# brunohs1993/Nanokappa

Measured on AMD Instinct MI355X. Metric: phonon-steps/sec (whole node), higher is better.
Workload: dtype f64

## Files before the change

include/nanokappa_hip.h:

```cpp
#ifndef NANOKAPPA_HIP_H
#define NANOKAPPA_HIP_H
#include <stdint.h>

#ifdef __cplusplus
extern "C" {
#endif

typedef struct nk_ctx nk_ctx;

enum nk_status {
    NK_OK = 0,
    NK_ERR_HIP = -1,
    NK_ERR_ARG = -2,
    NK_ERR_CAPACITY = -3,
    NK_ERR_COMM = -4,
    NK_ERR_NODEVICE = -5
};

typedef struct {
    int32_t Q, J, NT;
    const double *omega;
    const double *group_vel;
    const double *T_grid;
    const double *lifetime;
// ... 54 lines not shown
    const int64_t *n_leaving;
} nk_reservoirs;

typedef struct {
    int32_t Fr;
    const int32_t *facet;
    const double *specularity;
    const uint8_t *true_spec;
    const int32_t *spec_map;
    const double *roulette;
    const int32_t *degen_j2;
} nk_rough;

typedef struct {
    double dt;
    int32_t norm_fixed;
    double particle_density;
    int32_t T_ref_local;
    double T_ref;
    int32_t flux_every;
    int32_t contains_every;
    int32_t track_ids;
} nk_params;

typedef struct {
    double *T_sv;
    double *E_sv;
    double *E_raw;
    double *N_sv;
    double *flux_raw;
    double *N_leaving;
    double *res_energy;
    double *res_flux;
    double *N_emitted;
} nk_tally;

typedef struct {
    double step_kernel_ms;
    double emit_kernel_ms;
    double events_kernel_ms;
    double total_ms;
    int64_t slots;
    int64_t live;
    int64_t regrows;
    int64_t halts;
    int64_t tau_rebuilds;
    int64_t batches;
    int64_t emit_fused;
    int64_t place_tries;
    double place_gbps;
    double place_worst_gbps;
    int64_t box_store;
} nk_timing;

int nk_device_count(void);
int nk_mesh_crossings(int device, int64_t n_rays, const double *origins, const double *dirs, int64_t n_faces, const double *v0,
                      const double *e1, const double *e2, int skip_self, int32_t *counts);
int nk_create(nk_ctx **out, int device_id, uint64_t seed);
void nk_destroy(nk_ctx *ctx);
const char *nk_last_error(const nk_ctx *ctx);

int nk_set_material(nk_ctx *ctx, const nk_material *m);
int nk_set_mesh(nk_ctx *ctx, const nk_mesh *m);
int nk_set_subvolumes(nk_ctx *ctx, const nk_subvols *s, const double *T_sv_init );
int nk_set_reservoirs(nk_ctx *ctx, const nk_reservoirs *r);
int nk_set_rough(nk_ctx *ctx, const nk_rough *r);
int nk_set_params(nk_ctx *ctx, const nk_params *p);

int nk_reserve(nk_ctx *ctx, int64_t capacity);
int nk_upload_particles(nk_ctx *ctx, int64_t N, const double *x, const double *y, const double *z,
                        const int32_t *mode, const double *occ, const double *n_ts, const int32_t *facet,
                        const uint64_t *pid, uint64_t pid_offset);
int nk_init_boundaries(nk_ctx *ctx);
int nk_init_particles(nk_ctx *ctx, int64_t N, int64_t capacity, uint64_t pid_lo, const int32_t *unique_modes, int64_t n_unique,
                      const int64_t *sv_first);
int nk_tally_state(nk_ctx *ctx, double *E_raw, double *N_sv, double *flux_raw);
int nk_step(nk_ctx *ctx, int32_t nsteps, nk_tally *out);
int nk_download_particles(nk_ctx *ctx, int64_t capacity, double *x, double *y, double *z, int32_t *mode,
                          double *occ, double *n_ts, int32_t *facet, uint64_t *pid, int64_t *N_out);
int nk_get_subvol_temperature(nk_ctx *ctx, double *T_sv );
int nk_set_subvol_temperature(nk_ctx *ctx, const double *T_sv );
int nk_get_step(nk_ctx *ctx, int64_t *step);
int nk_get_timing(nk_ctx *ctx, nk_timing *t);

int nk_comm_unique_id(void *id128 );
int nk_comm_init(nk_ctx *ctx, const void *id128, int rank, int nranks);
typedef struct {
    int32_t rank, nranks;
    int32_t comm_rank, comm_nranks;
    int32_t device;
    int32_t selftest_ok;
    double selftest_sum;
    char pci_bus_id[32];
} nk_comm_report;
int nk_comm_info(nk_ctx *ctx, nk_comm_report *out);
int nk_comm_allreduce(nk_ctx *ctx, double *inout, int64_t n);

int nk_set_bands(nk_ctx *ctx, int32_t nbands, const int32_t *band_of_mode);
int nk_get_band_rows(nk_ctx *ctx, double *F, double *N, int64_t *steps, int32_t cap, int32_t *nrows);
int nk_tally_bands_state(nk_ctx *ctx, double *F, double *N);

typedef struct {
    double lo[3], h[3];
    int32_t n[3];
    int32_t every;
    int32_t flags;
    int64_t capacity;
} nk_field;
#define NK_FIELD_GLOBAL 1
#define NK_FIELD_TEST_SMALL_BOUND 2
int nk_set_field(nk_ctx *ctx, const nk_field *f);
int nk_get_field(nk_ctx *ctx, double *N, double *E, double *F, int64_t *samples, int64_t *clamped, int32_t reset);
int nk_tally_field_state(nk_ctx *ctx, int64_t *raw, int64_t *clamped);
typedef struct {
    int32_t n[3], every;
    int64_t ncells;
    int32_t k_E, k_F;
    double B_E, B_F;
    int64_t capacity;
    int64_t bytes;
    int32_t lds_path;
    int32_t on;
} nk_field_report;
int nk_field_info(nk_ctx *ctx, nk_field_report *out);

int nk_set_field_groups(nk_ctx *ctx, int32_t ngroups, const int32_t *group_of_mode);
int nk_get_field_groups(nk_ctx *ctx, double *N, double *E, double *F, int64_t *samples, int64_t *ungrouped, int32_t reset);
int nk_tally_field_groups_state(nk_ctx *ctx, int64_t *raw, int64_t *clamped, int64_t *ungrouped);
typedef struct {
    int32_t G;
    int32_t lds_path;
    int64_t lines;
    int64_t bytes;
    int32_t k_E, k_F;
    int64_t permutes;
    int32_t on, pad_;
} nk_field_groups_report;
int nk_field_groups_info(nk_ctx *ctx, nk_field_groups_report *out);

typedef struct {
    int64_t ncells, pairs;
    int32_t k_A, k_P;
    double seconds;
} nk_solid_report;
int nk_cell_solid_volume(int device, int64_t n_faces, const double *tri , const double lo[3],
                         const double h[3], const int32_t n[3], double *V , nk_solid_report *rep );
const char *nk_solid_last_error(void);

typedef struct {
    int32_t every;
    int32_t flags;
    int64_t capacity;
} nk_modes;
#define NK_MODES_GLOBAL 1
#define NK_MODES_TEST_SMALL_BOUND 2
int nk_set_modes(nk_ctx *ctx, const nk_modes *m);
int nk_get_modes(nk_ctx *ctx, double *N, double *E, int64_t *samples, int64_t *skipped, int32_t reset);
int nk_tally_modes_state(nk_ctx *ctx, int64_t *N, int64_t *E);
typedef struct {
    int32_t every, k_E;
    double B_E;
    int64_t capacity;
    int64_t bytes;
    int32_t owner_path;
    int32_t on;
} nk_modes_report;
// ... 192 lines not shown
```

nanokappa_amd/csrc/nk_engine.hip:

```cpp
#include <hip/hip_runtime.h>
#include <dlfcn.h>
#include <math.h>
#include <stdio.h>
#include <stdlib.h>
#include <string.h>
#include <algorithm>
#include <functional>
#include <map>
#include <mutex>
#include <queue>
#include <string>
#include <type_traits>
#include <chrono>
#include <time.h>
#include <vector>

#include <rccl/rccl.h>

#include "../../include/nanokappa_hip.h"
#include "nk_kernels.h"
#include "nk_field.h"
#include "nk_modes.h"
#include "nk_group.h"
#include "nk_freepath.h"
#include "nk_freecols.h"
#include "nk_kinetic.h"
#ifndef NK_PLAIN_IN_ENGINE
extern template __global__ void k_sweep<1, false, false, false, false, true, 1>(NkDev, uint32_t, int, int);
extern template __global__ void k_sweep<1, false, false, false, false, true, 2>(NkDev, uint32_t, int, int);
extern template __global__ void k_sweep<1, false, false, false, false, false, 1>(NkDev, uint32_t, int, int);
extern template __global__ void k_sweep<1, false, false, false, false, false, 2>(NkDev, uint32_t, int, int);
extern template __global__ void k_sweep<1, false, false, false, false, true, 1, true>(NkDev, uint32_t, int, int);
extern template __global__ void k_sweep<1, false, false, false, false, true, 2, true>(NkDev, uint32_t, int, int);
extern template __global__ void k_sweep<1, false, false, false, false, false, 1, true>(NkDev, uint32_t, int, int);
extern template __global__ void k_sweep<1, false, false, false, false, false, 2, true>(NkDev, uint32_t, int, int);
#endif

struct NkRccl {
    void *lib = nullptr;
    ncclResult_t (*GetUniqueId)(ncclUniqueId *) = nullptr;
    ncclResult_t (*CommInitRank)(ncclComm_t *, int, ncclUniqueId, int) = nullptr;
    ncclResult_t (*AllReduce)(const void *, void *, size_t, ncclDataType_t, ncclRedOp_t, ncclComm_t, hipStream_t) = nullptr;
    ncclResult_t (*CommDestroy)(ncclComm_t) = nullptr;
    ncclResult_t (*CommCount)(const ncclComm_t, int *) = nullptr;
    ncclResult_t (*CommUserRank)(const ncclComm_t, int *) = nullptr;
    ncclResult_t (*CommAbort)(ncclComm_t) = nullptr;
};

static thread_local std::string g_create_error;

struct nk_ctx {
    int device = 0;
    hipStream_t stream = nullptr;
    std::string err;
    NkDev d;
    std::vector<void *> allocs;
    std::vector<void *> pallocs;
    void *store_buf = nullptr;
    size_t store_pad = 0;
    bool store_pid = false;
    bool store_nts = true;
    bool mesh_box = false;
    bool box_forbidden = false;
    int32_t *anomalies = nullptr;
    bool have_material = false, have_mesh = false, have_sv = false, have_params = false;
    int64_t step = 0;
    bool pending_relax = false;
    int g_sweep = 0;
    std::vector<hipEvent_t> evpool;
    NkSweepKind g_sweep_kind = {};
    size_t g_sweep_lds = 0;
    int layout_key = -1;
    std::vector<double> h_enter_prob;
    int64_t spec_M = 0;
    double *spec_v = nullptr, *spec_om = nullptr, *spec_dl = nullptr, *spec_svx = nullptr;
    int32_t *spec_rank = nullptr;
    double spec_vmax = 0.0;
    NkSpecMode *spec_modes = nullptr;
    int32_t *spec_in = nullptr, *spec_out = nullptr;
    unsigned long long *spec_count = nullptr;
    double *ks_kv = nullptr, *ks_mat = nullptr;
    double ks_tol[3] = {0, 0, 0};
    int64_t ks_Q = 0;
    int64_t spec_cap = 0;
    int64_t spec_last = 0;
    int rb_Fr = 0;
    double *rb_k2 = nullptr, *rb_nin = nullptr, *rb_eta = nullptr, *rb_sub = nullptr, *rb_spec = nullptr, *rb_roul = nullptr;
    uint8_t *rb_ts = nullptr;
    unsigned int *rb_map = nullptr;
    std::vector<int32_t> rb_facet;
    int64_t o2o_first = 0;
    bool stepped = false;
    int64_t emitted_for = -1;
    std::vector<double> h_vg;
    std::vector<int32_t> h_m2s, h_s2m;
    int32_t *m2s_dev = nullptr, *s2m_dev = nullptr, *nl_dev = nullptr;
    unsigned int *rbar = nullptr;
    bool walked = false;
    int map_nseg = 0;
    NkMode *modetab_p = nullptr;
    int64_t modetab_p_len = 0;
    void *inbox = nullptr, *inbox_n = nullptr;
    void *mig_buf = nullptr, *mig_n = nullptr;
    double *ep_p = nullptr, *rc_p = nullptr;
    int rm_nseg = 0, rm_nlmax = 0;
    int32_t halt_words[4] = {0, 0, 0, 0};
    double *acc = nullptr;
    double *hist = nullptr;
    int hist_cap = 0;
    nk_params params;
    nk_timing timing;
    NkRccl rccl;
    ncclComm_t comm = nullptr;
    int comm_rank = -1, comm_nranks = 0;
    double comm_selftest = 0.0;
    int num_cu = 256;
    std::vector<int32_t> h_ffo, h_ffi;
    std::vector<double> h_fcdf, h_verts;
    std::vector<double> h_rbf_inv;
    std::vector<NkFacet> host_facets;
    const double *d_omega = nullptr, *d_vg = nullptr;
    std::vector<double> h_Tgrid;
    double T_lo = 0.0, T_hi = 0.0;
    int32_t band_B = 0;
    int32_t *band_map = nullptr;
    double *band_slabs = nullptr;
    size_t band_slabs_n = 0;
    double *band_rows_d = nullptr;
    size_t band_rows_n = 0;
    std::vector<double> band_rows;
    std::vector<int64_t> band_steps;
    NkFieldHost field;
    NkFGroupsHost fgroups;
    int64_t map_gen = 0;
    NkModesHost modes;
    double res_T_max = 0.0;
    nk_free_path_report fp_last = {};
    int32_t fc_calls = 0;
    int32_t kin_calls = 0;
    nk_free_path_map_report fm_last = {};
};

#define NK_HIP(call)                                                                                   \
    do {                                                                                               \
        hipError_t e_ = (call);                                                                        \
        if (e_ != hipSuccess) {                                                                        \
            ctx->err = std::string(#call) + ": " + hipGetErrorString(e_);                              \
            return NK_ERR_HIP;                                                                         \
        }                                                                                              \
    } while (0)
#define NK_ARG(cond, msg)                                                                              \
    do {                                                                                               \
        if (!(cond)) { ctx->err = msg; return NK_ERR_ARG; }                                            \
    } while (0)
#define NK_TRY(call)                                                                                   \
    do { int rc_ = (call); if (rc_) return rc_; } while (0)

template <class T>
static int nk_upload(nk_ctx *ctx, const T *src, size_t n, const T **dst, bool particle = false) {
    void *p = nullptr;
    size_t bytes = (n ? n : 1) * sizeof(T);
    NK_HIP(hipMalloc(&p, bytes));
    (particle ? ctx->pallocs : ctx->allocs).push_back(p);
    if (src && n) NK_HIP(hipMemcpy(p, src, n * sizeof(T), hipMemcpyHostToDevice));
    else NK_HIP(hipMemset(p, 0, bytes));
    *dst = (const T *)p;
    return NK_OK;
}
#define NK_UP(src, n, dst) NK_TRY(nk_upload(ctx, src, n, dst))
template <class T>
static int nk_palloc(nk_ctx *ctx, T *&field, size_t count) {
    const T *p = nullptr;
    NK_TRY(nk_upload<T>(ctx, nullptr, count, &p, true));
    field = (T *)p;
    return NK_OK;
}

static inline int nk_particle_bytes(bool with_pid, bool with_nts) { return 36 + (with_nts ? 8 : 0) + (with_pid ? 8 : 0); }
static inline size_t nk_store_bytes(int64_t cap, bool with_pid, bool with_nts) {
    const int64_t nblk = (cap + 63) / 64;
    const int nf = 4 + (with_nts ? 1 : 0) + (with_pid ? 1 : 0);
    const int bd = nf * 64 + 32;
    const size_t bytes = (size_t)nblk * bd * 8;
    return bytes ? bytes : 64;
}
static void nk_point_fields(NkDev &d, double *b, int64_t cap, bool with_pid, bool with_nts) {
    const int nf = 4 + (with_nts ? 1 : 0) + (with_pid ? 1 : 0);
// ... 127 lines not shown
int nk_device_count(void) {
    int ndev = 0;
    return hipGetDeviceCount(&ndev) == hipSuccess ? ndev : 0;
}

int nk_create(nk_ctx **out, int device_id, uint64_t seed) {
    if (!out) { g_create_error = "nk_create: out is NULL"; return NK_ERR_ARG; }
    *out = nullptr;
    int ndev = 0;
    hipError_t e = hipGetDeviceCount(&ndev);
    if (e != hipSuccess || ndev <= 0) {
        g_create_error = std::string("nk_create: no HIP device available (") + hipGetErrorString(e) +
                         "); this library has no CPU fallback";
        return NK_ERR_NODEVICE;
    }
    if (device_id < 0 || device_id >= ndev) { g_create_error = "nk_create: device_id out of range"; return NK_ERR_ARG; }
    nk_ctx *ctx = new nk_ctx();
    memset(&ctx->d, 0, sizeof(NkDev));
    memset(&ctx->params, 0, sizeof(nk_params));
    memset(&ctx->timing, 0, sizeof(nk_timing));
    ctx->device = device_id;
    if ((e = hipSetDevice(device_id)) != hipSuccess || (e = hipStreamCreate(&ctx->stream)) != hipSuccess) {
        g_create_error = std::string("nk_create: ") + hipGetErrorString(e);
        delete ctx;
        return NK_ERR_HIP;
    }
    hipDeviceProp_t prop;
    if (hipGetDeviceProperties(&prop, device_id) == hipSuccess) {
        ctx->num_cu = prop.multiProcessorCount;
        if (strncmp(prop.gcnArchName, "gfx950", 6) != 0) {
            g_create_error = std::string("nk_create: device is ") + prop.gcnArchName + ", this build targets gfx950 only";
            hipStreamDestroy(ctx->stream);
            delete ctx;
            return NK_ERR_NODEVICE;
        }
    }
    ctx->d.seed = seed;
    ctx->d.rank = 0;
    ctx->d.nranks = 1;
    ctx->d.tau_row0 = -1;
    ctx->d.stamps = nullptr;
    ctx->params.dt = 1.0; ctx->params.T_ref_local = 1; ctx->params.flux_every = 10; ctx->params.contains_every = 100;
    ctx->d.dt = 1.0; ctx->d.inv_dt = 1.0; ctx->d.T_ref_local = 1;
    const int32_t *p32 = nullptr;
    int rc;
    if ((rc = nk_upload<int32_t>(ctx, nullptr, 16, &p32))) {
        g_create_error = ctx->err;
        delete ctx;
        return rc;
    }
    ctx->d.halt = (int32_t *)p32;
    ctx->d.overflow = (int32_t *)p32 + 4;
    ctx->d.ticket = (int32_t *)p32 + 5;
    ctx->d.ev_ticket = (int32_t *)p32 + 6;
    ctx->anomalies = (int32_t *)p32 + 7;
    *out = ctx;
    return NK_OK;
}

static void nk_specular_free(nk_ctx *ctx);

void nk_destroy(nk_ctx *ctx) {
    if (!ctx) return;
    hipSetDevice(ctx->device);
    hipStreamSynchronize(ctx->stream);
    if (ctx->comm && ctx->rccl.CommDestroy) ctx->rccl.CommDestroy(ctx->comm);
    for (auto &e : ctx->evpool) hipEventDestroy(e);
    nk_specular_free(ctx);
    for (void *p : ctx->allocs) hipFree(p);
    for (void *p : ctx->pallocs) hipFree(p);
    if (ctx->acc) hipFree(ctx->acc);
    if (ctx->rbar) hipFree(ctx->rbar);
    if (ctx->hist) hipHostFree(ctx->hist);
    if (ctx->modetab_p) hipFree(ctx->modetab_p);
    if (ctx->m2s_dev) hipFree(ctx->m2s_dev);
    if (ctx->s2m_dev) hipFree(ctx->s2m_dev);
    if (ctx->nl_dev) hipFree(ctx->nl_dev);
    if (ctx->inbox) hipFree(ctx->inbox);
    if (ctx->inbox_n) hipFree(ctx->inbox_n);
    if (ctx->mig_buf) hipFree(ctx->mig_buf);
    if (ctx->mig_n) hipFree(ctx->mig_n);
    if (ctx->ep_p) hipFree(ctx->ep_p);
    if (ctx->rc_p) hipFree(ctx->rc_p);
    if (ctx->band_map) hipFree(ctx->band_map);
    if (ctx->band_slabs) hipFree(ctx->band_slabs);
    if (ctx->band_rows_d) hipFree(ctx->band_rows_d);
    nk_field_free(ctx->field);
    nk_fgroups_free(ctx->fgroups);
    nk_modes_free(ctx->modes);
    hipStreamDestroy(ctx->stream);
    delete ctx;
}

int nk_set_material(nk_ctx *ctx, const nk_material *m) {
    if (ctx) ctx->emitted_for = -1;
    NK_ARG(ctx && m, "nk_set_material: NULL argument");
    NK_ARG(m->Q > 0 && m->J > 0 && m->NT >= 2 && m->nE >= 2, "nk_set_material: bad sizes");
    NK_HIP(hipSetDevice(ctx->device));
    NkDev &d = ctx->d;
    d.Q = m->Q; d.J = m->J; d.NT = m->NT; d.M = m->Q * m->J;
    for (int i = 1; i < m->NT; ++i) NK_ARG(m->T_grid[i] > m->T_grid[i - 1], "nk_set_material: T_grid must ascend");
    NK_UP(m->omega, (size_t)d.M, &ctx->d_omega);
    NK_UP(m->group_vel, (size_t)d.M * 3, &ctx->d_vg);
    ctx->h_vg.assign(m->group_vel, m->group_vel + (size_t)d.M * 3);
    NK_UP((const NkMode *)nullptr, (size_t)d.M, &d.modetab);
    NK_UP(m->lifetime, (size_t)d.NT * d.M, &d.tau);
    NK_UP(m->T_grid, (size_t)d.NT, &d.Tgrid);
    ctx->h_Tgrid.assign(m->T_grid, m->T_grid + m->NT);
    d.nE = m->nE;
    NK_UP(m->T_array, (size_t)d.nE, &d.Tarr);
    NK_UP(m->energy_array, (size_t)d.nE, &d.Earr);
    d.Tfill_lo = m->T_fill_lo; d.Tfill_hi = m->T_fill_hi;
    d.hbar = m->hbar; d.kb = m->kb; d.QV = m->QV; d.active_modes = (double)m->active_modes;
    ctx->have_material = true;
    ctx->T_lo = ctx->T_hi = m->T_grid[0];
    int rc = nk_update_tau_window(ctx, true);
    if (rc) return rc;
    NK_HIP(hipStreamSynchronize(ctx->stream));
    return NK_OK;
}

struct NkFaceRef { int face; double lo[3], hi[3]; };
static int nk_clip_polygon(const double (*P)[3], int n, int axis, double c, bool upper, double (*out)[3]) {
    int no = 0;
    for (int i = 0; i < n; ++i) {
        const double *A = P[i], *B = P[(i + 1) % n];
        const bool ina = upper ? A[axis] >= c : A[axis] <= c, inb = upper ? B[axis] >= c : B[axis] <= c;
        if (ina) { for (int k = 0; k < 3; ++k) out[no][k] = A[k]; ++no; }
        if (ina != inb) {
            const double t = (c - A[axis]) / (B[axis] - A[axis]);
            for (int k = 0; k < 3; ++k) out[no][k] = A[k] + t * (B[k] - A[k]);
            out[no][axis] = c;
            ++no;
        }
    }
    return no;
}
static void nk_split_polygon(const double (*P)[3], int n, int face, int depth, std::vector<NkFaceRef> &refs) {
    NkFaceRef r;
    r.face = face;
    for (int k = 0; k < 3; ++k) { r.lo[k] = 1e300; r.hi[k] = -1e300; }
    for (int i = 0; i < n; ++i)
        for (int k = 0; k < 3; ++k) { r.lo[k] = std::min(r.lo[k], P[i][k]); r.hi[k] = std::max(r.hi[k], P[i][k]); }
    double area2[3] = {0, 0, 0};
    for (int i = 1; i + 1 < n; ++i) {
        double a[3], b[3];
        for (int k = 0; k < 3; ++k) { a[k] = P[i][k] - P[0][k]; b[k] = P[i + 1][k] - P[0][k]; }
        area2[0] += a[1] * b[2] - a[2] * b[1]; area2[1] += a[2] * b[0] - a[0] * b[2]; area2[2] += a[0] * b[1] - a[1] * b[0];
    }
    const double area = 0.5 * sqrt(area2[0] * area2[0] + area2[1] * area2[1] + area2[2] * area2[2]);
    const double e[3] = {r.hi[0] - r.lo[0], r.hi[1] - r.lo[1], r.hi[2] - r.lo[2]};
    const double box_area = e[0] * e[1] + e[1] * e[2] + e[0] * e[2];
    int axis = 0;
    for (int k = 1; k < 3; ++k) if (e[k] > e[axis]) axis = k;
    if (depth <= 0 || n < 3 || n > 12 || !(box_area > 3.0 * area) || !(e[axis] > 0.0)) { refs.push_back(r); return; }
    const double c = 0.5 * (r.lo[axis] + r.hi[axis]);
    double lo[16][3], hi[16][3];
    const int nl = nk_clip_polygon(P, n, axis, c, false, lo), nh = nk_clip_polygon(P, n, axis, c, true, hi);
    if (nl < 3 || nh < 3) { refs.push_back(r); return; }
    nk_split_polygon(lo, nl, face, depth - 1, refs);
    nk_split_polygon(hi, nh, face, depth - 1, refs);
}
static void nk_split_face(const double *V, int face, int max_depth, std::vector<NkFaceRef> &refs) {
    double P[16][3];
    for (int a = 0; a < 3; ++a) for (int k = 0; k < 3; ++k) P[a][k] = V[3 * a + k];
    nk_split_polygon(P, 3, face, max_depth, refs);
}

int nk_set_mesh(nk_ctx *ctx, const nk_mesh *m) {
    if (ctx) ctx->emitted_for = -1;
    NK_ARG(ctx && m, "nk_set_mesh: NULL argument");
    NK_ARG(m->F > 0 && m->Fc > 0, "nk_set_mesh: empty mesh");
    NK_HIP(hipSetDevice(ctx->device));
    NkDev &d = ctx->d;
    d.F = m->F; d.Fc = m->Fc; d.tol = m->tol;
    for (int i = 0; i < 6; ++i) d.bbox[i] = m->bbox[i];
    std::vector<std::vector<int>> members;
    for (int f = 0; f < m->F; ++f) {
        int found = -1;
        for (size_t pl = 0; pl < members.size() && found < 0; ++pl) {
            int g = members[pl][0];
            if (m->normals[3 * g] == m->normals[3 * f] && m->normals[3 * g + 1] == m->normals[3 * f + 1] &&
                m->normals[3 * g + 2] == m->normals[3 * f + 2] && m->k[g] == m->k[f])
                found = (int)pl;
        }
        if (found < 0) { members.push_back(std::vector<int>()); found = (int)members.size() - 1; }
        members[found].push_back(f);
    }
    d.NP = (int)members.size();
    std::vector<double> planes((size_t)d.NP * NK_PLANE_DOUBLES, 0.0), faces((size_t)m->F * NK_FACE_DOUBLES, 0.0);
    std::vector<int> face_pos((size_t)m->F, 0);
    int pos = 0;
    for (int pl = 0; pl < d.NP; ++pl) {
        double *p = &planes[(size_t)pl * NK_PLANE_DOUBLES];
        int g = members[pl][0];
        p[0] = m->normals[3 * g]; p[1] = m->normals[3 * g + 1]; p[2] = m->normals[3 * g + 2]; p[3] = m->k[g];
        int32_t rng[2] = {pos, pos + (int)members[pl].size()};
        memcpy(p + 4, rng, 8);
        for (int f : members[pl]) {
            double *q = &faces[(size_t)pos * NK_FACE_DOUBLES];
            for (int k = 0; k < 3; ++k) {
                q[k] = m->bounds_lo[3 * f + k]; q[3 + k] = m->bounds_hi[3 * f + k]; q[6 + k] = m->origins[3 * f + k];
            }
            const double *A = m->basis + 9 * f;
            double a00 = A[0], a01 = A[1], a02 = A[2], a10 = A[3], a11 = A[4], a12 = A[5], a20 = A[6], a21 = A[7], a22 = A[8];
            double det = a00 * (a11 * a22 - a12 * a21) - a01 * (a10 * a22 - a12 * a20) + a02 * (a10 * a21 - a11 * a20);
            NK_ARG(det != 0.0 && isfinite(det), "nk_set_mesh: degenerate face");
            q[9] = (a11 * a22 - a12 * a21) / det; q[10] = (a02 * a21 - a01 * a22) / det; q[11] = (a01 * a12 - a02 * a11) / det;
            q[12] = (a12 * a20 - a10 * a22) / det; q[13] = (a00 * a22 - a02 * a20) / det; q[14] = (a02 * a10 - a00 * a12) / det;
            int32_t id[2] = {f, m->face_facet[f]};
            memcpy(q + 15, id, 8);
            face_pos[f] = pos;
            ++pos;
        }
    }
    d.NG = 0;
    d.tree_top = 0; d.tree_leaves = 0;
    d.tree_nfam = 0; d.tree_lds_fam0 = 0; d.tree_lds_off = 0;
    for (int k = 0; k < NK_TREE_LEVELS; ++k) d.tree_base[k] = 0;
    bool use_tree = !(m->F <= NK_LDS_FACES && m->Fc <= NK_LDS_FACES) && !getenv("NK_NO_TREE");
    std::vector<NkFaceRef> refs;
    if (use_tree) {
        const int max_depth = getenv("NK_TREE_SPLIT") ? atoi(getenv("NK_TREE_SPLIT")) : 4;
        for (int f = 0; f < m->F; ++f) nk_split_face(m->vertices + 9 * (size_t)f, f, max_depth, refs);
        if (refs.size() > (size_t)4 * (1 << (2 * NK_TREE_LEVELS))) {
            refs.clear();
            for (int f = 0; f < m->F; ++f) nk_split_face(m->vertices + 9 * (size_t)f, f, 0, refs);
        }
        use_tree = refs.size() <= (size_t)4 * (1 << (2 * NK_TREE_LEVELS));
    }
    if (use_tree) {
        const int F = (int)refs.size();
        int top = 0;
        while ((int64_t)4 << (2 * top) < (int64_t)(F + 3) / 4) ++top;
        const int per_top = 1 << (2 * top);
        const int c_top = std::max(1, (int)(((int64_t)(F + 3) / 4 + per_top - 1) / per_top));
        const int NL = c_top * per_top;
        std::vector<int> order((size_t)F), slot((size_t)NL * 4, -1);
        for (int i = 0; i < F; ++i) order[i] = i;
        std::vector<double> cen((size_t)F * 3);
        for (int i = 0; i < F; ++i) for (int k = 0; k < 3; ++k) cen[3 * (size_t)i + k] = 0.5 * (refs[i].lo[k] + refs[i].hi[k]);
        std::function<void(int, int, const int *, int)> cut = [&](int a, int b, const int *sizes, int n) {
            if (n <= 1 || b - a <= 1) return;
            double lo[3] = {1e300, 1e300, 1e300}, hi[3] = {-1e300, -1e300, -1e300};
            for (int i = a; i < b; ++i)
                for (int k = 0; k < 3; ++k) { lo[k] = std::min(lo[k], cen[3 * (size_t)order[i] + k]); hi[k] = std::max(hi[k], cen[3 * (size_t)order[i] + k]); }
            int axis = 0;
            for (int k = 1; k < 3; ++k) if (hi[k] - lo[k] > hi[axis] - lo[axis]) axis = k;
            const int nl = n / 2;
            int left = 0;
            for (int i = 0; i < nl; ++i) left += sizes[i];
            if (left > 0 && left < b - a)
                std::nth_element(order.begin() + a, order.begin() + a + left, order.begin() + b, [&](int p, int q) {
// ... 177 lines not shown
            fs[2 * (size_t)fc + 1] = std::max(fs[2 * (size_t)fc + 1], dk);
        }
        std::vector<int> nfaces((size_t)m->Fc, 0);
        for (int f = 0; f < m->F; ++f) if (m->face_facet[f] >= 0 && m->face_facet[f] < m->Fc) ++nfaces[m->face_facet[f]];
        for (int fc = 0; fc < m->Fc; ++fc) if (nfaces[fc] < 16) fs[2 * (size_t)fc] = 1e300;
        NK_UP(fs.data(), fs.size(), &d.facet_skip);
    }
    d.nS = m->nS;
    if (m->nS > 0) {
        NK_UP(m->simplex_pts, (size_t)m->nS * 12, &d.simplex_pts);
        std::vector<double> sc((size_t)m->nS);
        double tot = 0.0, acc = 0.0;
        for (int s = 0; s < m->nS; ++s) tot += m->simplex_vol[s];
        for (int s = 0; s < m->nS; ++s) { acc += m->simplex_vol[s] / tot; sc[s] = acc; }
        for (int s = 0; s < m->nS; ++s) sc[s] /= sc[m->nS - 1];
        NK_UP(sc.data(), sc.size(), &d.simplex_cdf);
    }
    ctx->mesh_box = false;
    if (d.cap == 0) d.box = 0;
    if (m->F == 12 && m->Fc == 6 && d.NP == 6) {
        bool ok = true;
        int seen = 0;
        int box_facet[6] = {0, 0, 0, 0, 0, 0};
        d.box_ids = 0;
        for (int pl = 0; pl < 6 && ok; ++pl) {
            const double *pn = &planes[(size_t)pl * NK_PLANE_DOUBLES];
            int a = -1, sgn = 0;
            for (int k = 0; k < 3; ++k) {
                if (pn[k] == 1.0 || pn[k] == -1.0) { if (a >= 0) ok = false; a = k; sgn = pn[k] > 0 ? 1 : 0; }
                else if (pn[k] != 0.0) ok = false;
            }
            if (!ok || a < 0) { ok = false; break; }
            const int w = 2 * a + sgn;
            if (seen & (1 << w)) { ok = false; break; }
            seen |= 1 << w;
            const double wall = sgn ? -pn[3] : pn[3];
            if (!(fabs(wall - m->bbox[(sgn ? 3 : 0) + a]) <= 1e-9 * (1.0 + fabs(wall)))) { ok = false; break; }
            if (members[pl].size() != 2) { ok = false; break; }
            int fct0 = -1, face0 = 0x7fffffff;
            double area = 0.0;
            for (int f : members[pl]) {
                if (fct0 < 0) fct0 = m->face_facet[f]; else if (m->face_facet[f] != fct0) ok = false;
                face0 = std::min(face0, f);
                area += m->face_area[f];
                const double *V = m->vertices + 9 * (size_t)f;
                for (int c = 0; c < 3 && ok; ++c)
                    for (int k = 0; k < 3; ++k) {
                        const double v = V[3 * c + k], lo = m->bbox[k], hi = m->bbox[3 + k];
                        const double e = 1e-9 * (1.0 + fabs(lo) + fabs(hi));
                        if (k == a) { if (fabs(v - wall) > e) ok = false; }
                        else if (fabs(v - lo) > e && fabs(v - hi) > e) ok = false;
                    }
            }
            const int b = (a + 1) % 3, c = (a + 2) % 3;
            const double side = (m->bbox[3 + b] - m->bbox[b]) * (m->bbox[3 + c] - m->bbox[c]);
            if (!(fabs(area - side) <= 1e-9 * side) || fct0 < 0 || fct0 >= m->Fc) ok = false;
            if (!ok) break;
            d.box_k[w] = pn[3];
            box_facet[w] = fct0;
            d.box_ids = (d.box_ids & ~(0xFFull << (8 * w))) | ((uint64_t)(fct0 & 15) << (8 * w)) | ((uint64_t)(face0 & 15) << (8 * w + 4));
        }
        if (ok && seen == 63) {
            int fm = 0;
            for (int w = 0; w < 6; ++w) fm |= 1 << box_facet[w];
            ctx->mesh_box = fm == 63;
        }
    }
    ctx->have_mesh = true;
    return NK_OK;
}

static inline bool nk_want_box(const nk_ctx *ctx) {
    return ctx->have_mesh && ctx->mesh_box && !ctx->box_forbidden && !getenv("NK_NO_BOX") && !getenv("NK_SPLIT") &&
           ctx->d.F <= NK_LDS_FACES && ctx->d.Fc <= NK_LDS_FACES;
}

static int nk_patch_facets(nk_ctx *ctx) {
    NK_HIP(hipMemcpy((void *)ctx->d.facets, ctx->host_facets.data(), (size_t)ctx->d.Fc * sizeof(NkFacet), hipMemcpyHostToDevice));
    return NK_OK;
}

static int nk_entry_tables_drop(nk_ctx *ctx, bool keep_counters) {
    NkDev &d = ctx->d;
    if (ctx->rm_nseg > 0 && keep_counters && d.R > 0 && d.res_counter) {
        const int64_t n = (int64_t)d.R * d.M;
        k_perm_rm<<<(int)((n + 255) / 256), 256, 0, ctx->stream>>>(0, d.R, d.M, ctx->rm_nseg, ctx->rm_nlmax,
                                                                   d.m2s, d.res_counter, ctx->rc_p + (ctx->step & 1) * d.rc_len);
        NK_HIP(hipGetLastError());
        NK_HIP(hipStreamSynchronize(ctx->stream));
    }
    if (ctx->ep_p) { hipFree(ctx->ep_p); ctx->ep_p = nullptr; }
    if (ctx->rc_p) { hipFree(ctx->rc_p); ctx->rc_p = nullptr; }
    d.ep_p = nullptr; d.rc_p = nullptr;
    ctx->rm_nseg = 0;
    return NK_OK;
}
static int nk_entry_tables_build(nk_ctx *ctx) {
    NkDev &d = ctx->d;
    if (!(d.R > 0 && d.nseg > 0 && d.m2s && d.enter_prob && d.res_counter) || ctx->rm_nseg == d.nseg) return NK_OK;
    int rc = nk_entry_tables_drop(ctx, true);
    if (rc) return rc;
    const size_t len = (size_t)d.nseg * d.R * d.nlmax;
    NK_HIP(hipMalloc((void **)&ctx->ep_p, len * 8));
    NK_HIP(hipMalloc((void **)&ctx->rc_p, 2 * len * 8));
    NK_HIP(hipMemsetAsync(ctx->ep_p, 0, len * 8, ctx->stream));
    NK_HIP(hipMemsetAsync(ctx->rc_p, 0, 2 * len * 8, ctx->stream));
    d.rc_len = (int64_t)len;
    const int64_t n = (int64_t)d.R * d.M;
    k_perm_rm<<<(int)((n + 255) / 256), 256, 0, ctx->stream>>>(1, d.R, d.M, d.nseg, d.nlmax, d.m2s, (double *)d.enter_prob, ctx->ep_p);
    k_perm_rm<<<(int)((n + 255) / 256), 256, 0, ctx->stream>>>(1, d.R, d.M, d.nseg, d.nlmax, d.m2s, d.res_counter, ctx->rc_p + (ctx->step & 1) * d.rc_len);
    NK_HIP(hipGetLastError());
    d.ep_p = ctx->ep_p; d.rc_p = ctx->rc_p;
    ctx->rm_nseg = d.nseg;
    ctx->rm_nlmax = d.nlmax;
    return NK_OK;
}

static int nk_alloc_tally(nk_ctx *ctx) {
    NkDev &d = ctx->d;
    d.NB = 5 * d.S + 5 * d.R + 1;
    if (ctx->acc) { hipFree(ctx->acc); ctx->acc = nullptr; }
    if (ctx->hist) { hipHostFree(ctx->hist); ctx->hist = nullptr; }
    ctx->hist_cap = 0;
    NK_HIP(hipMalloc((void **)&ctx->acc, (size_t)(d.NB + 2) * sizeof(double)));
    NK_HIP(hipMemset(ctx->acc, 0, (size_t)(d.NB + 2) * sizeof(double)));
    const double *p;
    NK_UP((const double *)nullptr, (size_t)(ctx->num_cu * 16) * d.NB, &p);
    d.partials = (double *)p;
    return NK_OK;
}

static void nk_rbf_coefficients(nk_ctx *ctx, std::vector<double> &T) {
    const int S = ctx->d.S, P = ctx->d.rbf_P;
    T.resize((size_t)S + P);
    for (int j = 0; j < P; ++j) {
        double a = 0.0;
        for (int i = 0; i < S; ++i) a += ctx->h_rbf_inv[(size_t)j * P + i] * T[i];
        T[(size_t)S + j] = a;
    }
}

int nk_set_subvolumes(nk_ctx *ctx, const nk_subvols *s, const double *T_sv_init) {
    if (ctx) ctx->emitted_for = -1;
    NK_ARG(ctx && s && T_sv_init, "nk_set_subvolumes: NULL argument");
    NK_ARG(s->S > 0 && s->S <= 512, "nk_set_subvolumes: S must be in [1, 512]");
    NK_ARG(ctx->have_material, "nk_set_subvolumes: call nk_set_material first");
    NK_HIP(hipSetDevice(ctx->device));
    NkDev &d = ctx->d;
    d.S = s->S; d.sv_kind = s->kind; d.sv_axis = s->axis; d.sv_interp = s->interp;
    NK_ARG(s->axis >= 0 && s->axis < 3, "nk_set_subvolumes: axis");
    NK_ARG(!(s->kind != 0 && s->interp != 2 && s->interp != 3), "nk_set_subvolumes: slice interpolation needs slice subvolumes");
    NK_ARG(s->interp >= 0 && s->interp <= 3, "nk_set_subvolumes: interp must be 0..3");
    NK_UP(s->centers, (size_t)s->S * 3, &d.centers);
    NK_UP(s->volumes, (size_t)s->S, &d.sv_volume);
    d.rbf_P = 0;
    std::vector<double> t0(T_sv_init, T_sv_init + s->S);
    if (s->interp == 3) {
        NK_ARG(s->rbf_inv && s->rbf_shift && s->rbf_scale, "nk_set_subvolumes: interp 3 needs the RBF tables");
        const int nd = (s->rbf_used[0] != 0) + (s->rbf_used[1] != 0) + (s->rbf_used[2] != 0);
        NK_ARG(nd >= 1, "nk_set_subvolumes: RBF interpolation over no coordinate");
        d.rbf_P = s->S + nd + 1;
        for (int k = 0; k < 3; ++k) {
            d.rbf_used[k] = s->rbf_used[k] != 0; d.rbf_shift[k] = s->rbf_shift[k]; d.rbf_scale[k] = s->rbf_scale[k];
            NK_ARG(!d.rbf_used[k] || d.rbf_scale[k] != 0.0, "nk_set_subvolumes: zero RBF scale");
        }
        NK_UP(s->rbf_inv, (size_t)d.rbf_P * d.rbf_P, &d.rbf_inv);
        ctx->h_rbf_inv.assign(s->rbf_inv, s->rbf_inv + (size_t)d.rbf_P * d.rbf_P);
        nk_rbf_coefficients(ctx, t0);
    }
    const double *t;
    NK_UP(t0.data(), t0.size(), &t);
    d.T_sv = (double *)t;
    if (s->kind == 0 && s->S > 1) {
        double c0 = s->centers[s->axis], c1 = s->centers[3 + s->axis];
        NK_ARG(c1 > c0, "nk_set_subvolumes: slice centres must ascend along the axis");
        double Lx = c1 - c0;
        d.sv_lo = c0 - 0.5 * Lx; d.sv_invL = 1.0 / Lx;
    } else { d.sv_lo = 0.0; d.sv_invL = 0.0; }
    ctx->have_sv = true;
    nk_track_T(ctx, T_sv_init, s->S);
    int rc = nk_update_tau_window(ctx, false);
    if (rc) return rc;
    return nk_alloc_tally(ctx);
}

int nk_set_reservoirs(nk_ctx *ctx, const nk_reservoirs *r) {
    if (ctx) ctx->emitted_for = -1;
    NK_ARG(ctx && r, "nk_set_reservoirs: NULL argument");
    NK_ARG(ctx->have_material && ctx->have_mesh && ctx->have_sv, "nk_set_reservoirs: set material, mesh, subvolumes first");
    NK_ARG(r->R >= 0 && r->R <= 64, "nk_set_reservoirs: R must be in [0, 64]");
    NK_HIP(hipSetDevice(ctx->device));
    NkDev &d = ctx->d;
    NK_TRY(nk_entry_tables_drop(ctx, false));
    d.R = r->R; d.res_gen = r->gen;
    d.res_nf = 0; d.res_lds = 0;
    NK_ARG((int64_t)d.R * d.M < (1ll << 28), "nk_set_reservoirs: R*Q*J too large for the particle id layout");
    if (r->R > 0) {
        NK_UP(r->facet, (size_t)r->R, &d.res_facet);
        NK_UP(r->T, (size_t)r->R, &d.res_T);
        ctx->res_T_max = *std::max_element(r->T, r->T + r->R);
        NK_UP(r->enter_prob, (size_t)r->R * d.M, &d.enter_prob);
        const double *c;
        NK_UP(r->counter, (size_t)r->R * d.M, &c);
        d.res_counter = (double *)c;
        double pmax = 0.0;
        for (size_t i = 0; i < (size_t)r->R * d.M; ++i) pmax = std::max(pmax, r->enter_prob[i]);
        ctx->h_enter_prob.assign(r->enter_prob, r->enter_prob + (size_t)r->R * d.M);
        ctx->o2o_first = 0;
        NK_ARG(r->gen >= 0 && r->gen <= 2, "nk_set_reservoirs: gen must be 0 (constant), 1 (fixed_rate) or 2 (one_to_one)");
        if (r->gen == 2) {
            NK_ARG(r->n_leaving, "nk_set_reservoirs: one_to_one needs n_leaving");
            std::vector<double> roul((size_t)r->R * d.M);
            std::vector<int32_t> nl((size_t)r->R);
            int64_t first = 0;
            for (int i = 0; i < r->R; ++i) {
                double run = 0.0, mx = 0.0;
                for (int m = 0; m < d.M; ++m) { run += r->enter_prob[(size_t)i * d.M + m]; roul[(size_t)i * d.M + m] = run; mx = std::max(mx, run); }
                NK_ARG(mx > 0.0, "nk_set_reservoirs: one_to_one reservoir with zero entry probability");
                for (int m = 0; m < d.M; ++m) roul[(size_t)i * d.M + m] /= mx;
                NK_ARG(r->n_leaving[i] >= 0 && r->n_leaving[i] < (1ll << 24), "nk_set_reservoirs: n_leaving out of range");
                nl[(size_t)i] = (int32_t)r->n_leaving[i];
                first += r->n_leaving[i];
            }
            NK_UP(roul.data(), roul.size(), &d.res_roulette);
            const int32_t *pn;
            NK_UP(nl.data(), nl.size(), &pn);
            d.nleave_prev = (int32_t *)pn;
            ctx->o2o_first = first;
        }
        NK_ARG(pmax < 4094.0, "nk_set_reservoirs: more than 4094 particles of one mode per step (id layout)");
        for (int i = 0; i < r->R; ++i) {
            NK_ARG(r->facet[i] >= 0 && r->facet[i] < d.Fc, "nk_set_reservoirs: facet index");
            ctx->host_facets[r->facet[i]].res = i;
        }
        std::vector<int32_t> off((size_t)r->R + 1, 0);
        std::vector<double> rcdf, rverts;
        for (int i = 0; i < r->R; ++i) {
            const int f0 = ctx->h_ffo[r->facet[i]], f1 = ctx->h_ffo[r->facet[i] + 1];
            NK_ARG(f1 > f0, "nk_set_reservoirs: reservoir facet without faces");
            for (int a = f0; a < f1; ++a) {
                rcdf.push_back(ctx->h_fcdf[a]);
                const double *v = &ctx->h_verts[(size_t)ctx->h_ffi[a] * 9];
                rverts.insert(rverts.end(), v, v + 9);
            }
            off[(size_t)i + 1] = (int32_t)rcdf.size();
        }
        NK_UP(off.data(), off.size(), &d.res_face_off);
        NK_UP(rcdf.data(), rcdf.size(), &d.res_face_cdf);
        NK_UP(rverts.data(), rverts.size(), &d.res_face_verts);
        d.res_nf = (int32_t)rcdf.size();
        d.res_lds = d.res_nf <= NK_LDS_RESFACES ? 1 : 0;
        int rc = nk_patch_facets(ctx);
        if (rc) return rc;
        if ((rc = nk_entry_tables_build(ctx))) return rc;
    }
    return nk_alloc_tally(ctx);
}

int nk_set_rough(nk_ctx *ctx, const nk_rough *r) {
    if (ctx) ctx->emitted_for = -1;
    NK_ARG(ctx && r, "nk_set_rough: NULL argument");
    NK_ARG(ctx->have_material && ctx->have_mesh, "nk_set_rough: set material and mesh first");
    NK_HIP(hipSetDevice(ctx->device));
    NkDev &d = ctx->d;
    d.Fr = r->Fr;
    ctx->g_sweep = 0;
    if (r->Fr > 0) {
        size_t n = (size_t)r->Fr * d.M;
        NK_UP(r->specularity, n, &d.specularity);
        NK_UP(r->true_spec, n, &d.true_spec);
        NK_UP(r->spec_map, n, &d.spec_map);
        NK_UP(r->roulette, n, &d.roulette);
        {
            int nlut = 1024;
            while (nlut < 65536 && (int64_t)nlut * 4 < d.M) nlut *= 2;
            d.roul_nlut = nlut;
            std::vector<int32_t> lut((size_t)r->Fr * (nlut + 1));
            for (int f = 0; f < r->Fr; ++f) {
                const double *ro = r->roulette + (size_t)f * d.M;
                const double last = ro[d.M - 1];
                int pos = 0;
                for (int k = 0; k < nlut; ++k) {
                    const double thr = ((double)k / (double)nlut) * last;
                    while (pos < d.M && ro[pos] < thr) ++pos;
                    lut[(size_t)f * (nlut + 1) + k] = pos;
                }
                lut[(size_t)f * (nlut + 1) + nlut] = d.M;
            }
            NK_UP(lut.data(), lut.size(), &d.roul_lut);
        }
        if (r->degen_j2) NK_UP(r->degen_j2, (size_t)d.M, &d.degen_j2); else d.degen_j2 = nullptr;
        for (int i = 0; i < r->Fr; ++i) {
            NK_ARG(r->facet[i] >= 0 && r->facet[i] < d.Fc, "nk_set_rough: facet index");
            ctx->host_facets[r->facet[i]].rough = i;
        }
        return nk_patch_facets(ctx);
    }
    return NK_OK;
}

int nk_set_params(nk_ctx *ctx, const nk_params *p) {
    if (ctx) ctx->emitted_for = -1;
    NK_ARG(ctx && p, "nk_set_params: NULL argument");
    NK_ARG(p->dt > 0, "nk_set_params: dt must be positive");
    ctx->params = *p;
    NkDev &d = ctx->d;
    d.dt = p->dt; d.inv_dt = 1.0 / p->dt; d.norm_fixed = p->norm_fixed; d.particle_density = p->particle_density;
    d.T_ref_local = p->T_ref_local; d.T_ref = p->T_ref;
    ctx->have_params = true;
    return NK_OK;
}

struct NkHostParticles {
    std::vector<double> x, y, z, occ, nts;
    std::vector<int32_t> mode, facet;
    std::vector<uint64_t> pid;
};
static int nk_normalize(nk_ctx *ctx, int honor_halt = 0) {
    NkDev &d = ctx->d;
    d.down = 0;
    if (!ctx->walked || !d.seg_lo) return NK_OK;
    k_anchor<<<ctx->num_cu * 8, NK_WG, 0, ctx->stream>>>(d, honor_halt);
    NK_HIP(hipGetLastError());
    if (!honor_halt) ctx->walked = false;
    return NK_OK;
}
static int nk_gather_live(nk_ctx *ctx, NkHostParticles &h, bool want_all) {
    NkDev &d = ctx->d;
    if (d.cap == 0) return NK_OK;
    NK_TRY(nk_normalize(ctx));
    NK_HIP(hipStreamSynchronize(ctx->stream));
    std::vector<int32_t> cnt((size_t)d.nseg);
    NK_HIP(hipMemcpy(cnt.data(), d.seg_count, (size_t)d.nseg * 4, hipMemcpyDeviceToHost));
    int64_t live = 0;
    for (int c : cnt) live += c;
    if (!want_all) { h.x.resize((size_t)live); return NK_OK; }
    std::vector<double> bd;
    std::vector<uint32_t> bw;
    std::vector<uint64_t> bu;
    auto keep = [&](const auto &all, auto *dst) {
        for (int sgm = 0; sgm < d.nseg; ++sgm) {
            memcpy(dst, all.data() + (size_t)sgm * d.segcap, (size_t)cnt[sgm] * sizeof(*dst));
            dst += cnt[sgm];
        }
    };
    h.x.resize(live); h.y.resize(live); h.z.resize(live); h.occ.resize(live); h.nts.resize(live);
    h.mode.resize(live); h.facet.resize(live); h.pid.assign(live, 0);
    std::vector<uint32_t> w0((size_t)live);
    int rc;
    if ((rc = nk_field_download(ctx, d, d.x, bd))) return rc; keep(bd, h.x.data());
    if ((rc = nk_field_download(ctx, d, d.y, bd))) return rc; keep(bd, h.y.data());
    if ((rc = nk_field_download(ctx, d, d.z, bd))) return rc; keep(bd, h.z.data());
    if ((rc = nk_field_download(ctx, d, d.occ, bd))) return rc; keep(bd, h.occ.data());
    std::vector<int32_t> bfc;
    if (d.nts) { if ((rc = nk_field_download(ctx, d, d.nts, bd))) return rc; keep(bd, h.nts.data()); }
    else {
        if (ctx->have_material && ctx->have_mesh && ctx->have_sv && d.modetab) {
            double *dn = nullptr; int32_t *df = nullptr;
            NK_HIP(hipMalloc((void **)&dn, (size_t)d.cap * 8));
            if (hipMalloc((void **)&df, (size_t)d.cap * 4) != hipSuccess) { hipFree(dn); ctx->err = "nk_gather_live: out of memory"; return NK_ERR_HIP; }
            hipMemsetAsync(dn, 0, (size_t)d.cap * 8, ctx->stream); hipMemsetAsync(df, 0xff, (size_t)d.cap * 4, ctx->stream);
            k_next_hit<1><<<nk_sweep_grid(ctx), NK_WG, nk_lds(ctx, true), ctx->stream>>>(d, dn, df);
            bd.resize((size_t)d.cap); bfc.resize((size_t)d.cap);
            hipError_t e1 = hipGetLastError();
            if (e1 == hipSuccess) e1 = hipMemcpy(bd.data(), dn, (size_t)d.cap * 8, hipMemcpyDeviceToHost);
            if (e1 == hipSuccess) e1 = hipMemcpy(bfc.data(), df, (size_t)d.cap * 4, hipMemcpyDeviceToHost);
            hipFree(dn); hipFree(df);
            if (e1 != hipSuccess) { ctx->err = std::string("nk_gather_live: ") + hipGetErrorString(e1); return NK_ERR_HIP; }
            keep(bd, h.nts.data());
        } else { std::fill(h.nts.begin(), h.nts.end(), 0.0); }
    }
    if ((rc = nk_field_download(ctx, d, d.w0, bw))) return rc; keep(bw, w0.data());
    if (d.pid) { if ((rc = nk_field_download(ctx, d, d.pid, bu))) return rc; keep(bu, h.pid.data()); }
    const uint32_t lbmask = (1u << d.lb) - 1u;
    int64_t k = 0;
    for (int sgm = 0; sgm < d.nseg; ++sgm)
        for (int j = 0; j < cnt[sgm]; ++j, ++k) {
            const uint32_t idx = w0[(size_t)k] & lbmask;
            h.mode[(size_t)k] = d.part ? ctx->h_s2m[(size_t)sgm * d.nlmax + idx] : (int32_t)idx;
            if (d.nts) h.facet[(size_t)k] = (int32_t)(w0[(size_t)k] >> d.lb) - 1;
            else h.facet[(size_t)k] = (w0[(size_t)k] & NK_LOST) ? -1 : (bfc.empty() ? 0 : bfc[(size_t)sgm * d.segcap + j]);
        }
    return NK_OK;
}

// ... 46 lines not shown
            const uint32_t idx = d.part ? (uint32_t)(ctx->h_m2s[(size_t)mode[i]] / d.nseg) : (uint32_t)mode[i];
            w0[(size_t)i] = d.nts ? (((uint32_t)(fc + 1) << d.lb) | idx) : (((facet && fc < 0) ? NK_LOST : 0u) | idx);
        }
        if ((rc = put((const uint32_t *)w0.data(), d.w0))) return rc;
    }
    if (d.pid) {
        if (pid) { if ((rc = put(pid, d.pid))) return rc; }
        else {
            std::vector<uint64_t> ids((size_t)N);
            for (int64_t i = 0; i < N; ++i) ids[(size_t)i] = pid_offset + (uint64_t)i;
            if ((rc = put((const uint64_t *)ids.data(), d.pid))) return rc;
        }
    }
    NK_HIP(hipMemcpy(d.seg_count, cnt.data(), (size_t)d.nseg * 4, hipMemcpyHostToDevice));
    if (d.seg_lo) NK_HIP(hipMemset(d.seg_lo, 0, (size_t)d.nseg * 4));
    ctx->walked = false;
    return NK_OK;
}

static inline bool nk_want_pid(const nk_ctx *ctx) { return ctx->d.Fr > 0 || ctx->params.track_ids != 0; }
static inline bool nk_want_split(const nk_ctx *ctx) {
    if (const char *e = getenv("NK_SPLIT")) return atoi(e) != 0;
    return ctx->have_mesh && !(ctx->d.F <= NK_LDS_FACES && ctx->d.Fc <= NK_LDS_FACES);
}
static inline bool nk_want_part(const nk_ctx *ctx) { return !getenv("NK_NO_PARTITION"); }

static NkSweepKind nk_sweep_kind(const nk_ctx *ctx, bool stored) {
    const NkDev &d = ctx->d;
    return nk_kind_normalise({nk_geom_mode(ctx), d.Fr > 0, d.sv_interp == 3, stored ? (bool)d.pid : nk_want_pid(ctx),
                              stored ? d.qx != nullptr : nk_want_split(ctx), nk_want_lrec(ctx), nk_sweep_fast(ctx), d.box != 0});
}
typedef void (*NkSweepFn)(NkDev, uint32_t, int, int);
typedef void (*NkResidentFn)(NkDev, uint32_t, int, int, int, double *, int, unsigned int *);
static NkSweepFn nk_sweep_kernel(const NkSweepKind &k) {
    auto fast = [](auto L, auto F1, auto X) -> NkSweepFn { return k_sweep<1, false, false, false, false, L.value, F1.value ? 1 : 2, X.value>; };
    if (k.fast) return nk_lift(fast, k.lrec, k.fast == 1, k.box);
    return nk_lift([](auto G1, auto R, auto B, auto P, auto S, auto L, auto X) -> NkSweepFn {
        if constexpr ((R.value && !P.value) || (X.value && (!G1.value || S.value))) return nullptr;
        else return k_sweep<G1.value ? 1 : 2, R.value, B.value, P.value, S.value, L.value, 0, X.value>;
    }, k.geom == 1, k.rough, k.rbf, k.pid, k.split, k.lrec, k.box);
}
static NkSweepFn nk_events_kernel(const NkSweepKind &k) {
    return nk_lift([](auto G1, auto R, auto B, auto P) -> NkSweepFn {
        if constexpr (R.value && !P.value) return nullptr;
        else return k_events<G1.value ? 1 : 2, R.value, B.value, P.value>;
    }, k.geom == 1, k.rough, k.rbf, k.pid);
}
static NkResidentFn nk_resident_kernel(const NkSweepKind &k) {
    return nk_lift([](auto X, auto P, auto L) -> NkResidentFn { return k_resident<X.value, P.value, L.value>; }, k.box, k.pid, k.lrec);
}

static int nk_sweep_blocks(nk_ctx *ctx) {
    if (!(ctx->have_material && ctx->have_mesh && ctx->have_sv)) return ctx->num_cu * NK_SWEEP_OCC;
    const NkSweepKind kind = nk_sweep_kind(ctx, false);
    const size_t lds_w = nk_lds(ctx, true, kind.pid ? 3 : 2);
    if (ctx->g_sweep == 0 || !(ctx->g_sweep_kind == kind) || ctx->g_sweep_lds != lds_w) {
        int per_cu = 0;
        const NkSweepFn sweep = nk_sweep_kernel(kind);
        hipError_t e_ = sweep ? hipOccupancyMaxActiveBlocksPerMultiprocessor(&per_cu, sweep, NK_WG, lds_w) : hipErrorInvalidDeviceFunction;
        if (e_ != hipSuccess || per_cu < 1) per_cu = 1;
        if (per_cu > 8) per_cu = 8;
        { const int bound = NK_SWEEP_BOUND(kind.geom, kind.rough, kind.rbf, kind.split); if (per_cu > bound) per_cu = bound; }
        if (const char *e = getenv("NK_SWEEP_PER_CU")) { int v = atoi(e); if (v >= 1 && v < per_cu) per_cu = v; }
        ctx->g_sweep = ctx->num_cu * per_cu;
        ctx->g_sweep_kind = kind;
        ctx->g_sweep_lds = lds_w;
        if (getenv("NK_VERBOSE")) fprintf(stderr, "[nanokappa_hip] sweep: %d workgroups per CU (occupancy query rc %d), %zu B LDS each\n", per_cu, (int)e_, lds_w);
    }
    return ctx->g_sweep;
}

static inline int nk_mode_seg(const nk_ctx *ctx, int m, int nseg) {
    return (ctx->map_nseg == nseg && !ctx->h_m2s.empty()) ? ctx->h_m2s[(size_t)m] % nseg : m % nseg;
}

static int nk_build_mode_map(nk_ctx *ctx) {
    NkDev &d = ctx->d;
    if (ctx->m2s_dev) { hipFree(ctx->m2s_dev); ctx->m2s_dev = nullptr; }
    if (ctx->s2m_dev) { hipFree(ctx->s2m_dev); ctx->s2m_dev = nullptr; }
    if (ctx->nl_dev) { hipFree(ctx->nl_dev); ctx->nl_dev = nullptr; }
    d.m2s = nullptr; d.s2m = nullptr; d.seg_nl = nullptr;
    ctx->h_m2s.clear(); ctx->h_s2m.clear(); ctx->map_nseg = 0;
    ctx->map_gen += 1;
    if (d.M <= 0 || d.nseg <= 0) return NK_OK;
    const int M = d.M, nseg = d.nseg, nlmax = d.nlmax;
    const bool plain = !d.part;
    std::vector<int32_t> nl((size_t)nseg, 0);
    ctx->h_m2s.assign((size_t)M, 0);
    ctx->h_s2m.assign((size_t)nseg * nlmax, -1);
    auto place = [&](int m, int seg) {
        const int l = nl[(size_t)seg]++;
        ctx->h_m2s[(size_t)m] = l * nseg + seg;
        ctx->h_s2m[(size_t)seg * nlmax + l] = m;
    };
    if (plain) {
        for (int m = 0; m < M; ++m) place(m, m % nseg);
    } else {
        std::vector<double> rate((size_t)M, 0.0);
        std::vector<char> active((size_t)M, 1);
        const bool have_v = ctx->h_vg.size() == (size_t)M * 3;
        if (have_v) {
            double inv[3] = {0, 0, 0};
            if (ctx->have_mesh) for (int a = 0; a < 3; ++a) { const double e = d.bbox[3 + a] - d.bbox[a]; inv[a] = e > 0.0 ? 1.0 / e : 0.0; }
            for (int m = 0; m < M; ++m) {
                const double *v = &ctx->h_vg[3 * (size_t)m];
                active[(size_t)m] = (v[0] != 0.0 || v[1] != 0.0 || v[2] != 0.0) ? 1 : 0;
                rate[(size_t)m] = fabs(v[0]) * inv[0] + fabs(v[1]) * inv[1] + fabs(v[2]) * inv[2];
            }
        }
        double rsum = 0.0; int64_t nact = 0;
        for (int m = 0; m < M; ++m) if (active[(size_t)m]) { rsum += rate[(size_t)m]; ++nact; }
        const double rmean = nact > 0 && rsum > 0.0 ? rsum / (double)nact : 1.0;
        const double beta = getenv("NK_EVENT_WEIGHT") ? atof(getenv("NK_EVENT_WEIGHT")) : 0.45;
        std::vector<double> share((size_t)nseg, 1.0);
        const int g = ctx->g_sweep, per_cu = ctx->num_cu > 0 ? g / ctx->num_cu : 0;
        const double skew = getenv("NK_AGE_SKEW") ? atof(getenv("NK_AGE_SKEW")) : 0.14;
        if (per_cu > 1 && g == per_cu * ctx->num_cu && nseg == g * (NK_WG / 64) && skew != 0.0)
            for (int sg = 0; sg < nseg; ++sg) {
                const int k = (sg / (NK_WG / 64)) / ctx->num_cu;
                share[(size_t)sg] = 1.0 + skew * (1.0 - 2.0 * (double)k / (double)(per_cu - 1));
            }
        std::vector<int32_t> order((size_t)M);
        for (int m = 0; m < M; ++m) order[(size_t)m] = m;
        std::stable_sort(order.begin(), order.end(), [&](int32_t a, int32_t b) {
            if (active[(size_t)a] != active[(size_t)b]) return active[(size_t)a] > active[(size_t)b];
            return rate[(size_t)a] > rate[(size_t)b];
        });
        typedef std::pair<double, int> Key;
        std::priority_queue<Key, std::vector<Key>, std::greater<Key>> heap;
        std::vector<double> load((size_t)nseg, 0.0);
        for (int sg = 0; sg < nseg; ++sg) heap.push(Key(0.0, sg));
        int k = 0;
        for (; k < M && active[(size_t)order[(size_t)k]]; ++k) {
            const int m = order[(size_t)k];
            int sg = -1;
            while (!heap.empty()) { const Key top = heap.top(); heap.pop(); if (nl[(size_t)top.second] < nlmax) { sg = top.second; break; } }
            if (sg < 0) { ctx->err = "nk_build_mode_map: the segments' slot ranges are full (internal sizing error)"; return NK_ERR_ARG; }
            place(m, sg);
            load[(size_t)sg] += 1.0 + beta * rate[(size_t)m] / rmean;
            heap.push(Key(load[(size_t)sg] / share[(size_t)sg], sg));
        }
        std::priority_queue<std::pair<int, int>, std::vector<std::pair<int, int>>, std::greater<std::pair<int, int>>> room;
        for (int sg = 0; sg < nseg; ++sg) room.push(std::make_pair((int)nl[(size_t)sg], sg));
        for (; k < M; ++k) {
            const std::pair<int, int> top = room.top(); room.pop();
            if (top.first >= nlmax) { ctx->err = "nk_build_mode_map: no room for the inactive modes (internal sizing error)"; return NK_ERR_ARG; }
            place(order[(size_t)k], top.second);
            room.push(std::make_pair(top.first + 1, top.second));
        }
    }
    NK_HIP(hipMalloc((void **)&ctx->m2s_dev, (size_t)M * 4));
    NK_HIP(hipMalloc((void **)&ctx->s2m_dev, (size_t)nseg * nlmax * 4));
    NK_HIP(hipMalloc((void **)&ctx->nl_dev, (size_t)nseg * 4));
    NK_HIP(hipMemcpy(ctx->m2s_dev, ctx->h_m2s.data(), (size_t)M * 4, hipMemcpyHostToDevice));
    NK_HIP(hipMemcpy(ctx->s2m_dev, ctx->h_s2m.data(), (size_t)nseg * nlmax * 4, hipMemcpyHostToDevice));
    NK_HIP(hipMemcpy(ctx->nl_dev, nl.data(), (size_t)nseg * 4, hipMemcpyHostToDevice));
    d.m2s = ctx->m2s_dev; d.s2m = ctx->s2m_dev; d.seg_nl = ctx->nl_dev;
    ctx->map_nseg = nseg;
    return NK_OK;
}

static int64_t nk_spawn_bound(const nk_ctx *ctx, int nseg) {
    const NkDev &d = ctx->d;
    if (d.R <= 0) return 0;
    if (d.res_gen == 2) return 4 * (ctx->o2o_first / std::max(nseg, 1) + 64);
    std::vector<int64_t> per((size_t)nseg, 0);
// ... 647 lines not shown
static size_t nk_events_lds(nk_ctx *ctx, size_t lds_g) {
    NkDev &d = ctx->d;
    size_t lds_ev = lds_g;
    if (!(d.qx && nk_geom_mode(ctx) == 2 && d.NG > 0 && d.tree_nfam > 0)) return lds_ev;
    const size_t off = (lds_g + 15) & ~(size_t)15, fixed = off + (size_t)NK_EVENTS_PEND * NK_EV_WG * 4 + 1024;
    size_t budget = (size_t)160 * 1024 / NK_EV_PER_CU > fixed ? (size_t)160 * 1024 / NK_EV_PER_CU - fixed : 0;
    if (const char *e = getenv("NK_EVENTS_TREE_LDS")) { const size_t v = (size_t)atol(e); if (v < budget) budget = v; }
    for (int l = 0; l <= d.tree_top; ++l) {
        const int fam0 = d.tree_base[l] >> 2;
        const size_t bytes = (size_t)(d.tree_nfam - fam0) * NK_TREE_FAMILY_FLOATS * 4;
        if (bytes <= budget) { d.tree_lds_fam0 = fam0; d.tree_lds_off = (int32_t)off; lds_ev = off + bytes; break; }
    }
    if (getenv("NK_VERBOSE") && ctx->timing.batches <= 1)
        fprintf(stderr, "[nanokappa_hip] k_events: families %d .. %d of the face tree in LDS (%zu B of %zu B per workgroup)\n", d.tree_lds_fam0, d.tree_nfam, lds_ev - off, lds_ev);
    return lds_ev;
}
static int nk_side_tallies(nk_ctx *ctx, int s, std::vector<int> &band_s) {
    const int64_t stepno = ctx->step + s;
    if (!nk_flux_step(ctx, stepno)) return NK_OK;
    const int nranks = ctx->comm ? ctx->comm_nranks : 1;
    if (ctx->band_B > 0) {
        NK_TRY(nk_band_pass(ctx, false, ctx->band_rows_d + band_s.size() * 4 * (size_t)ctx->d.S * ctx->band_B));
        band_s.push_back(s);
    }
    if (ctx->field.on && nk_nth_step(ctx->field.cfg.every, stepno)) {
        NK_TRY(nk_field_sample(ctx, false, false));
        NK_HIP(nk_field_accumulate(ctx->field.g, ctx->field, nranks, ctx->stream));
        if (ctx->fgroups.on) {
            NK_TRY(nk_field_sample(ctx, true, false));
            NK_HIP(nk_field_accumulate(ctx->fgroups.g, ctx->field, nranks, ctx->stream));
        }
    }
    if (ctx->modes.on && nk_nth_step(ctx->modes.cfg.every, stepno)) {
        NK_TRY(nk_modes_sample(ctx, false));
        NK_HIP(nk_modes_accumulate(ctx->modes, nranks, ctx->num_cu, ctx->stream));
    }
    return NK_OK;
}
static int nk_band_collect(nk_ctx *ctx, const std::vector<int> &band_s, int32_t nd) {
    if (band_s.empty()) return NK_OK;
    const size_t rl = 4 * (size_t)ctx->d.S * ctx->band_B;
    std::vector<double> br(band_s.size() * rl);
    NK_HIP(hipMemcpyAsync(br.data(), ctx->band_rows_d, br.size() * sizeof(double), hipMemcpyDeviceToHost, ctx->stream));
    NK_HIP(hipStreamSynchronize(ctx->stream));
    const int unseen = ctx->halt_words[2] ? nd - 1 : -1;
    for (size_t r = 0; r < band_s.size(); ++r) {
        if (band_s[r] >= nd || band_s[r] == unseen) continue;
        ctx->band_rows.insert(ctx->band_rows.end(), br.begin() + r * rl, br.begin() + (r + 1) * rl);
        ctx->band_steps.push_back(ctx->step + band_s[r]);
    }
    return NK_OK;
}
static int nk_batch_timing(nk_ctx *ctx, int nev, int32_t nsteps, int32_t nd) {
    const hipEvent_t *ev = ctx->evpool.data();
    float ms = 0.f;
    double sk = 0.0, ek = 0.0, vk = 0.0;
    const int nt = nd < nev ? nd : nev;
    for (int s = 0; s < nt; ++s) {
        NK_HIP(hipEventElapsedTime(&ms, ev[4 * s], ev[4 * s + 1])); ek += ms;
        NK_HIP(hipEventElapsedTime(&ms, ev[4 * s + 1], ev[4 * s + 2])); sk += ms;
        NK_HIP(hipEventElapsedTime(&ms, ev[4 * s + 2], ev[4 * s + 3])); vk += ms;
    }
    NK_HIP(hipEventElapsedTime(&ms, ev[64], ev[65]));
    if (nt > 0 && nd == nsteps) {
        ctx->timing.step_kernel_ms = sk / nt;
        ctx->timing.emit_kernel_ms = ek / nt;
        ctx->timing.events_kernel_ms = vk / nt;
        ctx->timing.total_ms = ms;
    }
    return NK_OK;
}
#ifdef NK_STAMPS
#include "nk_stamps.h"
#endif
static int nk_wait_call(hipStream_t stream, int32_t nsteps, std::string &err) {
    hipError_t e = hipSuccess;
    const char *what = "hipStreamQuery";
    if (nsteps <= 4) while ((e = hipStreamQuery(stream)) == hipErrorNotReady) { }
    if (e == hipSuccess) { what = "hipStreamSynchronize(stream)"; e = hipStreamSynchronize(stream); }
    if (e != hipSuccess) { err = std::string(what) + ": " + hipGetErrorString(e); return NK_ERR_HIP; }
    return NK_OK;
}

static int nk_step_batch(nk_ctx *ctx, int32_t nsteps, std::vector<double> &h, int32_t *done) {
    NkDev &d = ctx->d;
    const int R = d.R, NB = d.NB;
    NkBatch b;
    NK_TRY(nk_batch_enter(ctx, nsteps, b));
    const size_t lds_g = nk_lds(ctx, true), lds_w = nk_lds(ctx, true, d.pid ? 3 : 2), lds_e = nk_lds(ctx, true, 1), lds_t = nk_tail_lds(ctx);
    const size_t lds_ev = nk_events_lds(ctx, lds_g);
    const NkSweepKind kind = nk_sweep_kind(ctx, true);
    const NkSweepFn sweep = nk_sweep_kernel(kind), events = kind.split ? nk_events_kernel(kind) : nullptr;
    NK_ARG(sweep && (events || !kind.split), "nk_step: no k_sweep / k_events is built for this configuration");
    if (kind.split) NK_HIP(nk_allow_lds((const void *)events, lds_ev));
    const int g_sweep = b.g_sweep, g_emit = b.g_emit;
    const int g_ev = kind.split ? ctx->num_cu * NK_EV_PER_CU : 0;
    const int rows = g_sweep + g_ev;
    const int nev = nsteps < 4 ? 0 : 4;
    NK_TRY(nk_batch_events(ctx));
    hipEvent_t *ev = ctx->evpool.data();
    NK_HIP(hipEventRecord(ev[64], ctx->stream));
    std::vector<int> band_s;
    if (ctx->band_B > 0) {
        int nflux = 0;
        for (int s = 0; s < nsteps; ++s) nflux += nk_flux_step(ctx, ctx->step + s) ? 1 : 0;
        if (nflux > 0) NK_TRY(nk_band_ensure(ctx, nflux));
    }
    for (int s = 0; s < nsteps; ++s) {
        NK_TRY(nk_batch_prelude(ctx, b, s));
        const NkGroupRec rec = nk_batch_rec(ctx, b, s);
        const uint32_t step = rec.step;
        const int do_flux = rec.do_flux;
        if (s < nev) NK_HIP(hipEventRecord(ev[4 * s], ctx->stream));
        if (R > 0 && d.res_gen == 2) k_emit_one_to_one<<<ctx->num_cu * 4, NK_WG, 0, ctx->stream>>>(d, step);
        if (R > 0 && !b.emitted_ahead) NK_EMIT_LAUNCH(k_emit, g_emit, lds_e, d, step);
        if (s < nev) NK_HIP(hipEventRecord(ev[4 * s + 1], ctx->stream));
        if (b.alt) ctx->walked = true;
        d.down = rec.down;
        sweep<<<g_sweep, NK_WG, lds_w, ctx->stream>>>(d, step, rec.do_relax, do_flux);
        d.down = 0;
        if (kind.split) {
            k_events_begin<<<1, 1024, 0, ctx->stream>>>(d);
            events<<<g_ev, NK_EV_WG, lds_ev, ctx->stream>>>(d, step, do_flux, g_sweep);
            k_events_end<<<(d.nseg + 255) / 256, 256, 0, ctx->stream>>>(d);
        }
        if (d.mig_buf) k_deliver<<<g_emit, NK_WG, 0, ctx->stream>>>(d, 1);
        if (s < nev) NK_HIP(hipEventRecord(ev[4 * s + 2], ctx->stream));
        NK_TRY(nk_side_tallies(ctx, s, band_s));
        double *hrow = rec.hist_row;
        const bool ahead = b.tail_emit;
        if (ctx->comm) {
            if (ahead) NK_EMIT_LAUNCH(k_tail, NB + g_emit, lds_t, d, step + 1u, rows, ctx->acc, hrow, do_flux, 0, NB);
            else k_reduce<<<NB, NK_WG, 0, ctx->stream>>>(d, rows, ctx->acc, hrow, do_flux, 0);
            ncclResult_t nrc = ctx->rccl.AllReduce(ctx->acc, ctx->acc, (size_t)NB + 2, ncclDouble, ncclSum, ctx->comm, ctx->stream);
            if (nrc != ncclSuccess) { ctx->err = "ncclAllReduce failed"; return NK_ERR_COMM; }
            k_update<<<1, NK_WG, 0, ctx->stream>>>(d, ctx->acc, hrow, do_flux);
        } else if (ahead) {
            NK_EMIT_LAUNCH(k_tail, NB + g_emit, lds_t, d, step + 1u, rows, ctx->acc, hrow, do_flux, 1, NB);
        } else {
            k_reduce<<<NB, NK_WG, 0, ctx->stream>>>(d, rows, ctx->acc, hrow, do_flux, 1);
        }
        b.emitted_ahead = ahead;
        if (s < nev) NK_HIP(hipEventRecord(ev[4 * s + 3], ctx->stream));
        if ((s & 63) == 0) NK_HIP(hipGetLastError());
    }
    NK_HIP(hipEventRecord(ev[65], ctx->stream));
    NK_HIP(hipGetLastError());
    NK_TRY(nk_wait_call(ctx->stream, nsteps, ctx->err));
    NK_TRY(nk_batch_collect(ctx, nsteps, h, done));
#ifdef NK_STAMPS
    NK_TRY(nk_stamps_report(ctx));
#endif
    NK_TRY(nk_band_collect(ctx, band_s, *done));
    nk_batch_leave(ctx, b, nsteps, *done);
    return nk_batch_timing(ctx, nev, nsteps, *done);
}

static inline bool nk_want_resident(const nk_ctx *ctx) {
    const NkDev &d = ctx->d;
    if (!getenv("NK_RESIDENT") || getenv("NK_NO_RESIDENT") || ctx->comm || d.nranks != 1 || d.Fr > 0 || d.mig_buf || d.qx || nk_geom_mode(ctx) != 1) return false;
    if (ctx->band_B > 0) return false;
    if (ctx->field.on) return false;
    if (ctx->modes.on) return false;
    if (d.res_gen == 2 || d.sv_interp == 3 || d.NB > 254 || d.S > 128 || d.nseg <= 0) return false;
    const int64_t lim = getenv("NK_RESIDENT_MAX") ? atoll(getenv("NK_RESIDENT_MAX")) : 1200000;
    return d.cap <= lim && nk_lds(ctx, true, 5) <= 160 * 1024;
}
static int nk_step_resident(nk_ctx *ctx, int32_t nsteps, std::vector<double> &h, int32_t *done) {
    NkDev &d = ctx->d;
    const int NB = d.NB;
    NkBatch b;
    NK_TRY(nk_batch_enter(ctx, nsteps, b, true));
    const NkSweepKind kind = nk_sweep_kind(ctx, true);
    const NkResidentFn resident = nk_resident_kernel(kind);
    NK_ARG(resident, "nk_step: no k_resident is built for this configuration");
    const size_t lds = nk_lds(ctx, true, kind.pid ? 5 : 4);
    if (nk_allow_lds((const void *)resident, lds) != hipSuccess) (void)hipGetLastError();
    int per_cu = 1;
    if (hipOccupancyMaxActiveBlocksPerMultiprocessor(&per_cu, resident, NK_WG, lds) != hipSuccess || per_cu < 1) { (void)hipGetLastError(); per_cu = 1; }
    if (per_cu > 2) per_cu = 2;
    int G = std::min(ctx->num_cu * per_cu, (d.nseg + NK_WG / 64 - 1) / (NK_WG / 64));
    if (const char *e = getenv("NK_RESIDENT_GRID")) { const int v = atoi(e); if (v >= 1 && v < G) G = v; }
    G = std::max(1, G);
    NK_ARG((size_t)2 * G * (size_t)((NB + 1) & ~1) <= (size_t)ctx->num_cu * 16 * NB, "nk_step_resident: tally rows exceed the partials buffer");
    NK_TRY(nk_batch_events(ctx));
    hipEvent_t t0 = ctx->evpool[64], t1 = ctx->evpool[65];
    if (!ctx->rbar) NK_HIP(hipMalloc((void **)&ctx->rbar, (32 + 4096) * sizeof(unsigned int)));
    NK_HIP(hipEventRecord(t0, ctx->stream));
    for (int k = 0; k < nsteps;) {
        NK_TRY(nk_batch_prelude(ctx, b, k));
        const NkGroupRec rec = nk_batch_rec(ctx, b, k);
        int n = 1;
        while (k + n < nsteps && !nk_contains_step(ctx, ctx->step + k + n)) ++n;
        NK_HIP(hipMemsetAsync(ctx->rbar, 0, (32 + 1024 + 128) * sizeof(unsigned int), ctx->stream));
        resident<<<G, NK_WG, lds, ctx->stream>>>(d, rec.step, n, rec.do_relax, ctx->params.flux_every, rec.hist_row, nk_row(ctx).width(), ctx->rbar);
        NK_HIP(hipGetLastError());
        k += n;
    }
    NK_HIP(hipEventRecord(t1, ctx->stream));
    NK_HIP(hipStreamSynchronize(ctx->stream));
    NK_TRY(nk_batch_collect(ctx, nsteps, h, done));
    const int32_t nd = *done;
    if (getenv("NK_VERBOSE") && ctx->timing.batches % 8 == 2) {
        unsigned long long m[12];
        NK_HIP(hipMemcpy(m, ctx->rbar + 8, sizeof(m), hipMemcpyDeviceToHost));
        if (m[0] && m[6] >= m[0])
            fprintf(stderr, "[nanokappa_hip] resident step, workgroup 0 [us]: sweep %.2f  row + flag %.2f  emission %.2f  all flags seen %.2f  rows summed %.2f  update published %.2f | workgroup G/2: sweep %.2f  row + emission %.2f  update seen %.2f\n",
                    (m[1] - m[0]) * 0.01, (m[2] - m[1]) * 0.01, (m[3] - m[2]) * 0.01, (m[4] - m[3]) * 0.01, (m[5] - m[4]) * 0.01, (m[6] - m[5]) * 0.01,
                    (m[9] - m[8]) * 0.01, (m[10] - m[9]) * 0.01, (m[11] - m[10]) * 0.01);
    }
    nk_batch_leave(ctx, b, nsteps, nd);
    float ms = 0.f;
    NK_HIP(hipEventElapsedTime(&ms, t0, t1));
    if (nd == nsteps && nd > 0) {
        ctx->timing.step_kernel_ms = (double)ms / nd;
        ctx->timing.emit_kernel_ms = 0.0;
        ctx->timing.events_kernel_ms = 0.0;
        ctx->timing.total_ms = ms;
    }
    return NK_OK;
}

static int nk_tallies_refresh(nk_ctx *ctx) {
    if (ctx->field.on) NK_TRY(nk_field_refresh(ctx));
    if (ctx->fgroups.on) NK_TRY(nk_fgroups_refresh(ctx));
    if (ctx->modes.on) NK_TRY(nk_modes_refresh(ctx));
    return NK_OK;
}
static int nk_step_begin(nk_ctx *ctx) {
    int rc = nk_check_ready(ctx);
    if (rc) return rc;
    NK_HIP(hipSetDevice(ctx->device));
    if ((rc = nk_update_tau_window(ctx, false))) return rc;
    if ((rc = nk_ensure_inbox(ctx))) return rc;
    if ((rc = nk_ensure_migration(ctx, 0))) return rc;
    ctx->stepped = true;
    ctx->band_rows.clear();
// ... 400 lines not shown
    for (int r = 0; r < R; ++r) { own[(size_t)r] = g->m[r]->stream; g->m[r]->stream = stream; }
    auto leave = [&](int code) { for (int r = 0; r < R; ++r) g->m[r]->stream = own[(size_t)r]; return code; };
    for (int r = 0; r < R; ++r)
        if ((rc = nk_step_begin(g->m[r]))) return leave(nk_member_failed(g, r, rc));
    std::vector<std::vector<double>> hs((size_t)R);
    std::vector<int32_t> nds((size_t)R, 0);
    if ((rc = nk_group_batch(g, plan, stream, nsteps, hs, nds))) return leave(rc);
    g->rep.steps += nsteps;
    for (int r = 0; r < R; ++r) {
        nk_ctx *ctx = g->m[r];
        NkStepRun run;
        nk_tally *out = outs ? &outs[r] : nullptr;
        const int64_t halts0 = ctx->timing.halts;
        if ((rc = nk_step_consume(ctx, nsteps, out, run, hs[(size_t)r], nds[(size_t)r]))) return leave(nk_member_failed(g, r, rc));
        if (ctx->timing.halts != halts0 && !g->halted[(size_t)r]) { g->halted[(size_t)r] = 1; g->rep.halted += 1; }
        if (run.s_out < nsteps) {
            if (!g->alone[(size_t)r]) { g->alone[(size_t)r] = 1; g->rep.finished_alone += 1; }
            std::vector<double> h;
            while (run.s_out < nsteps) {
                int32_t nd = 0;
                if ((rc = nk_step_batch(ctx, nsteps - run.s_out, h, &nd)) || (rc = nk_step_consume(ctx, nsteps, out, run, h, nd))) return leave(nk_member_failed(g, r, rc));
                g->rep.member_launches += 2 * (int64_t)nd;
            }
        }
        if ((rc = nk_step_end(ctx, run.overflow))) return leave(nk_member_failed(g, r, rc));
    }
    return leave(NK_OK);
}

int nk_download_particles(nk_ctx *ctx, int64_t capacity, double *x, double *y, double *z, int32_t *mode, double *occ,
                          double *n_ts, int32_t *facet, uint64_t *pid, int64_t *N_out) {
    NK_ARG(ctx && N_out, "nk_download_particles: NULL argument");
    NK_HIP(hipSetDevice(ctx->device));
    NkDev &d = ctx->d;
    *N_out = 0;
    if (d.cap == 0) return NK_OK;
    if (ctx->have_material && ctx->have_sv && ctx->have_mesh) NK_TRY(nk_flush_relax(ctx, 0));
    NkHostParticles h;
    int rc = nk_gather_live(ctx, h, capacity != 0);
    if (rc) return rc;
    const int64_t live = (int64_t)h.x.size();
    *N_out = live;
    if (capacity == 0) return NK_OK;
    NK_ARG(capacity >= live, "nk_download_particles: capacity smaller than the live particle count");
    if (x) memcpy(x, h.x.data(), live * 8);
    if (y) memcpy(y, h.y.data(), live * 8);
    if (z) memcpy(z, h.z.data(), live * 8);
    if (occ) memcpy(occ, h.occ.data(), live * 8);
    if (n_ts) memcpy(n_ts, h.nts.data(), live * 8);
    if (mode) memcpy(mode, h.mode.data(), live * 4);
    if (facet) memcpy(facet, h.facet.data(), live * 4);
    if (pid) memcpy(pid, h.pid.data(), live * 8);
    return NK_OK;
}

int nk_get_subvol_temperature(nk_ctx *ctx, double *T_sv) {
    NK_ARG(ctx && T_sv && ctx->have_sv, "nk_get_subvol_temperature: bad arguments");
    NK_HIP(hipSetDevice(ctx->device));
    NK_HIP(hipStreamSynchronize(ctx->stream));
    NK_HIP(hipMemcpy(T_sv, ctx->d.T_sv, (size_t)ctx->d.S * 8, hipMemcpyDeviceToHost));
    return NK_OK;
}
int nk_set_subvol_temperature(nk_ctx *ctx, const double *T_sv) {
    NK_ARG(ctx && T_sv && ctx->have_sv, "nk_set_subvol_temperature: bad arguments");
    NK_HIP(hipSetDevice(ctx->device));
    NK_HIP(hipStreamSynchronize(ctx->stream));
    std::vector<double> t(T_sv, T_sv + ctx->d.S);
    if (ctx->d.sv_interp == 3) nk_rbf_coefficients(ctx, t);
    NK_HIP(hipMemcpy(ctx->d.T_sv, t.data(), t.size() * 8, hipMemcpyHostToDevice));
    nk_track_T(ctx, T_sv, ctx->d.S);
    return NK_OK;
}
int nk_get_step(nk_ctx *ctx, int64_t *step) {
    NK_ARG(ctx && step, "nk_get_step: NULL argument");
    *step = ctx->step;
    return NK_OK;
}
int nk_get_timing(nk_ctx *ctx, nk_timing *t) {
    NK_ARG(ctx && t, "nk_get_timing: NULL argument");
    *t = ctx->timing;
    t->box_store = (ctx->d.cap > 0 && ctx->d.box) ? 1 : 0;
    return NK_OK;
}

static int nk_load_rccl(NkRccl &r, std::string &err) {
    if (r.lib) return NK_OK;
    const char *names[] = {"librccl.so.1", "librccl.so", "/opt/rocm/lib/librccl.so.1", "/opt/rocm/lib/librccl.so"};
    for (const char *n : names) { r.lib = dlopen(n, RTLD_NOW | RTLD_GLOBAL); if (r.lib) break; }
    if (!r.lib) { err = std::string("cannot load librccl: ") + dlerror(); return NK_ERR_COMM; }
    r.GetUniqueId = (decltype(r.GetUniqueId))dlsym(r.lib, "ncclGetUniqueId");
    r.CommInitRank = (decltype(r.CommInitRank))dlsym(r.lib, "ncclCommInitRank");
    r.AllReduce = (decltype(r.AllReduce))dlsym(r.lib, "ncclAllReduce");
    r.CommDestroy = (decltype(r.CommDestroy))dlsym(r.lib, "ncclCommDestroy");
    r.CommCount = (decltype(r.CommCount))dlsym(r.lib, "ncclCommCount");
    r.CommUserRank = (decltype(r.CommUserRank))dlsym(r.lib, "ncclCommUserRank");
    r.CommAbort = (decltype(r.CommAbort))dlsym(r.lib, "ncclCommAbort");
    if (!r.GetUniqueId || !r.CommInitRank || !r.AllReduce || !r.CommDestroy || !r.CommCount || !r.CommUserRank) { err = "librccl lacks expected symbols"; return NK_ERR_COMM; }
    return NK_OK;
}
int nk_comm_unique_id(void *id128) {
    static NkRccl r;
    std::string err;
    if (!id128) return NK_ERR_ARG;
    if (nk_load_rccl(r, err)) { g_create_error = err; return NK_ERR_COMM; }
    ncclUniqueId id;
    memset(&id, 0, sizeof(id));
    if (r.GetUniqueId(&id) != ncclSuccess) { g_create_error = "ncclGetUniqueId failed"; return NK_ERR_COMM; }
    memcpy(id128, &id, 128);
    return NK_OK;
}
int nk_comm_init(nk_ctx *ctx, const void *id128, int rank, int nranks) {
    if (ctx) ctx->emitted_for = -1;
    NK_ARG(ctx && id128 && nranks >= 1 && rank >= 0 && rank < nranks, "nk_comm_init: bad arguments");
    NK_ARG(!ctx->stepped, "nk_comm_init: must be called before the first nk_step (emission ownership is per rank)");
    NK_HIP(hipSetDevice(ctx->device));
    ctx->d.rank = rank;
    ctx->d.nranks = nranks;
    if (nranks == 1 && !getenv("NK_FORCE_COMM")) return NK_OK;
    if (getenv("NK_COMM_DRYRUN")) return NK_OK;
    if (nk_load_rccl(ctx->rccl, ctx->err)) return NK_ERR_COMM;
    ncclUniqueId id;
    static_assert(sizeof(ncclUniqueId) == 128, "ncclUniqueId is expected to be 128 bytes");
    memcpy(&id, id128, 128);
    auto fail = [&](const std::string &why, bool hung) -> int {
        ctx->err = why;
        if (ctx->comm) {
            if (hung && ctx->rccl.CommAbort) ctx->rccl.CommAbort(ctx->comm);
            else if (!hung && ctx->rccl.CommDestroy) ctx->rccl.CommDestroy(ctx->comm);
        }
        ctx->comm = nullptr; ctx->comm_rank = -1; ctx->comm_nranks = 0; ctx->comm_selftest = 0.0;
        ctx->d.rank = 0; ctx->d.nranks = 1;
        return NK_ERR_COMM;
    };
    if (ctx->rccl.CommInitRank(&ctx->comm, nranks, id, rank) != ncclSuccess) { ctx->comm = nullptr; return fail("ncclCommInitRank failed", false); }
    int cn = 0, cr = -1;
    if (ctx->rccl.CommCount(ctx->comm, &cn) != ncclSuccess || ctx->rccl.CommUserRank(ctx->comm, &cr) != ncclSuccess) {
        return fail("ncclCommCount / ncclCommUserRank failed", false);
    }
    ctx->comm_nranks = cn; ctx->comm_rank = cr;
    if (cn != nranks || cr != rank) {
        return fail("RCCL reports rank " + std::to_string(cr) + " of " + std::to_string(cn) + ", expected rank " + std::to_string(rank) + " of " + std::to_string(nranks), false);
    }
    double *probe = nullptr, hp[2] = {1.0, (double)(rank + 1)};
    double *hpin = nullptr;
    if (hipMalloc((void **)&probe, 16) != hipSuccess || hipHostMalloc((void **)&hpin, 16, hipHostMallocDefault) != hipSuccess) {
        if (probe) hipFree(probe);
        return fail("self-test of the new communicator: out of memory", false);
    }
    hpin[0] = hp[0]; hpin[1] = hp[1];
    hipError_t he = hipMemcpyAsync(probe, hpin, 16, hipMemcpyHostToDevice, ctx->stream);
    ncclResult_t nrc = he == hipSuccess ? ctx->rccl.AllReduce(probe, probe, 2, ncclDouble, ncclSum, ctx->comm, ctx->stream) : ncclSystemError;
    if (he == hipSuccess && nrc == ncclSuccess) he = hipMemcpyAsync(hpin, probe, 16, hipMemcpyDeviceToHost, ctx->stream);
    bool hung = false;
    if (he == hipSuccess && nrc == ncclSuccess) {
        const double limit = getenv("NK_COMM_TIMEOUT_S") ? atof(getenv("NK_COMM_TIMEOUT_S")) : 180.0;
        const auto t0 = std::chrono::steady_clock::now();
        for (;;) {
            he = hipStreamQuery(ctx->stream);
            if (he != hipErrorNotReady) break;
            if (std::chrono::duration<double>(std::chrono::steady_clock::now() - t0).count() > limit) { hung = true; break; }
            struct timespec ts = {0, 200000};
            nanosleep(&ts, nullptr);
        }
    }
    if (hung) return fail("self-test all-reduce of the new communicator did not finish in time: a rank is missing", true);
    hp[0] = hpin[0]; hp[1] = hpin[1];
    hipFree(probe); hipHostFree(hpin);
    if (he != hipSuccess || nrc != ncclSuccess) return fail("self-test all-reduce of the new communicator failed", false);
    ctx->comm_selftest = hp[0];
    if (hp[0] != (double)nranks || hp[1] != 0.5 * (double)nranks * (double)(nranks + 1)) {
        return fail("self-test all-reduce returned " + std::to_string(hp[0]) + " / " + std::to_string(hp[1]) + " instead of " +
                    std::to_string(nranks) + " / " + std::to_string(nranks * (nranks + 1) / 2) + ": not every rank took part", false);
    }
    return NK_OK;
}
int nk_comm_allreduce(nk_ctx *ctx, double *inout, int64_t n) {
    NK_ARG(ctx && inout && n >= 0, "nk_comm_allreduce: bad arguments");
    if (!ctx->comm || n == 0) return NK_OK;
    NK_HIP(hipSetDevice(ctx->device));
    double *buf = nullptr;
    NK_HIP(hipMalloc((void **)&buf, (size_t)n * 8));
    hipError_t he = hipMemcpyAsync(buf, inout, (size_t)n * 8, hipMemcpyHostToDevice, ctx->stream);
    ncclResult_t nrc = he == hipSuccess ? ctx->rccl.AllReduce(buf, buf, (size_t)n, ncclDouble, ncclSum, ctx->comm, ctx->stream) : ncclSystemError;
    if (he == hipSuccess && nrc == ncclSuccess) he = hipMemcpyAsync(inout, buf, (size_t)n * 8, hipMemcpyDeviceToHost, ctx->stream);
    if (he == hipSuccess && nrc == ncclSuccess) he = hipStreamSynchronize(ctx->stream);
    hipFree(buf);
    if (he != hipSuccess || nrc != ncclSuccess) { ctx->err = "nk_comm_allreduce failed"; return NK_ERR_COMM; }
    return NK_OK;
}
int nk_comm_info(nk_ctx *ctx, nk_comm_report *out) {
    NK_ARG(ctx && out, "nk_comm_info: NULL argument");
    memset(out, 0, sizeof(*out));
    out->rank = ctx->d.rank; out->nranks = ctx->d.nranks;
    out->comm_rank = ctx->comm ? ctx->comm_rank : -1;
    out->comm_nranks = ctx->comm ? ctx->comm_nranks : 0;
// ... 1207 lines not shown
```

nanokappa_amd/csrc/nk_kernels.h:

```cpp
#pragma once
#ifndef NK_KERNEL_LINKAGE
#define NK_KERNEL_LINKAGE
#endif
#include "nk_device.h"

#define NK_TILE 64
#ifndef NK_NT
#define NK_NT 0
#endif
#if NK_NT
#define NK_LD(p) __builtin_nontemporal_load(p)
#define NK_ST(p, v) __builtin_nontemporal_store(v, p)
#else
#define NK_LD(p) (*(p))
#define NK_ST(p, v) (*(p) = (v))
#endif
#ifdef NK_STAMPS
#define NK_STAMP(k)                                                                                    \
    do {                                                                                               \
        unsigned long long t_;                                                                         \
        __builtin_amdgcn_sched_barrier(0);                                                             \
        asm volatile("s_memtime %0\n\ts_waitcnt lgkmcnt(0)" : "=s"(t_)::"memory");                     \
        __builtin_amdgcn_sched_barrier(0);                                                             \
        st_acc[k] += t_ - st_last;                                                                     \
// ... 1298 lines not shown
    const double Ta = d.Tarr[0], Tb = d.Tarr[1], Tz = d.Tarr[n - 1], Ea = d.Earr[0], Ez = d.Earr[n - 1];
    for (int t = tid; t < S; t += nth) {
        double Tnew, E;
        nk_update_sv(d, acc[t], acc[S + t], d.T_ref_local ? d.T_sv[t] : d.T_ref, t, Ta, Tb, Tz, Ea, Ez, Tnew, E);
        hist_row[NB + t] = Tnew;
        hist_row[NB + S + t] = E;
        d.T_sv[t] = Tnew;
    }
    for (int b = tid; b < NB; b += nth) hist_row[b] = acc[b];
    if (d.sv_interp == 3) {
        __syncthreads();
        const int P = d.rbf_P;
        for (int j = tid; j < P; j += nth) {
            double a = 0.0;
            for (int i = 0; i < S; ++i) a += d.rbf_inv[(int64_t)j * P + i] * d.T_sv[i];
            d.T_sv[S + j] = a;
        }
    }
    if (d.res_gen == 2) for (int r = tid; r < d.R; r += nth) d.nleave_prev[r] = (int32_t)acc[5 * S + r];
    if (tid == 0) {
        hist_row[NB + 2 * S + 0] = (double)do_flux;
        hist_row[NB + 2 * S + 1] = 1.0;
        const bool hdel = acc[NB + 1] > 0.0;
        const bool hreq = acc[NB] > 0.0 || hdel;
        hist_row[NB + 2 * S + 2] = hreq ? 1.0 : 0.0;
        hist_row[NB + 2 * S + 3] = (double)*d.overflow;
        if (hreq) d.halt[0] = 1;
        if (hdel) d.halt[2] = 1;
        hist_row[NB + 2 * S + 4] = hreq ? 1.0 : 0.0;
        hist_row[NB + 2 * S + 5] = (double)d.halt[1];
        hist_row[NB + 2 * S + 6] = (hdel || d.halt[2]) ? 1.0 : 0.0;
        hist_row[NB + 2 * S + 7] = (double)d.halt[3];
    }
}

__device__ __forceinline__ void nk_reduce_body(const NkDev &d, int rows, double *acc, double *hist_row, int do_flux, int fuse, int b,
                                               int nblocks, double *sh, int &last) {
    if (d.halt[0]) return;
    const int NB = d.NB;
    double v = 0.0;
    for (int r = threadIdx.x; r < rows; r += NK_WG) v += d.partials[(int64_t)r * NB + b];
    sh[threadIdx.x] = v;
    __syncthreads();
    for (int o = NK_WG / 2; o > 0; o >>= 1) {
        if (threadIdx.x < o) sh[threadIdx.x] += sh[threadIdx.x + o];
        __syncthreads();
    }
    if (threadIdx.x == 0) acc[b] = sh[0];
    if (b == 0) {
        int stuck = 0;
        if (d.mig_n) for (int sg = threadIdx.x; sg < d.nseg; sg += NK_WG) { const int n = d.mig_n[sg]; stuck |= (n > 0 && d.seg_count[sg] + (n < d.mig_cap ? n : d.mig_cap) > d.segcap) ? 1 : 0; }
        stuck = __syncthreads_or(stuck);
        if (threadIdx.x == 0) { acc[NB] = (double)d.halt[1]; acc[NB + 1] = (double)stuck; }
    }
    if (!fuse) return;
    if (threadIdx.x == 0) {
        __threadfence();
        last = (atomicAdd(d.ticket, 1) == nblocks - 1);
    }
    __syncthreads();
    if (!last) return;
    if (threadIdx.x == 0) *d.ticket = 0;
    __threadfence();
    nk_update_body(d, acc, hist_row, do_flux);
}
NK_KERNEL_LINKAGE __global__ __launch_bounds__(NK_WG) void k_reduce(NkDev d, int rows, double *acc, double *hist_row, int do_flux, int fuse) {
    __shared__ double sh[NK_WG];
    __shared__ int last;
    nk_reduce_body(d, rows, acc, hist_row, do_flux, fuse, (int)blockIdx.x, (int)gridDim.x, sh, last);
}
template <int GEOM, bool BOX = false>
__global__ __launch_bounds__(NK_WG) void k_tail(NkDev d, uint32_t step_next, int rows, double *acc, double *hist_row, int do_flux, int fuse,
                                                int n_reduce) {
    extern __shared__ __align__(16) unsigned char smem[];
    if ((int)blockIdx.x < n_reduce) {
        double *sh = reinterpret_cast<double *>(smem);
        int &last = *reinterpret_cast<int *>(smem + NK_WG * sizeof(double));
        nk_reduce_body(d, rows, acc, hist_row, do_flux, fuse, (int)blockIdx.x, n_reduce, sh, last);
    } else {
        nk_emit_body<GEOM, BOX>(d, step_next, smem, (int)blockIdx.x - n_reduce, (int)gridDim.x - n_reduce, true);
    }
}

__device__ __forceinline__ bool nk_wait_word(const unsigned int *w, unsigned int atleast) {
    int spins = 0;
    while (__hip_atomic_load(w, __ATOMIC_RELAXED, __HIP_MEMORY_SCOPE_AGENT) < atleast) {
        __builtin_amdgcn_s_sleep(1);
        if (++spins > 1000000) return false;
    }
    return true;
}
template <bool BOX, bool PID, bool LREC>
__global__ __launch_bounds__(NK_WG, 2) void k_resident(NkDev d, uint32_t step0, int nsteps, int relax0, int flux_every, double *hist, int hrow,
                                                       unsigned int *bar) {
    extern __shared__ __align__(16) unsigned char smem[];
    if (d.halt[0]) return;
    NkLds L;
    nk_lds_setup<1, PID ? 5 : 4>(d, smem, L);
    const int tid = threadIdx.x, wg = (int)blockIdx.x, G = (int)gridDim.x;
    const int S = d.S, R = d.R, NB = d.NB, a = d.sv_axis;
    double *Tsv = const_cast<double *>(L.tb.Tsv);
    NkSv *sv = const_cast<NkSv *>(L.tb.sv);
    const int nE = d.nE;
    const double Ta = d.Tarr[0], Tb = d.Tarr[1], Tz = d.Tarr[nE - 1], Ea = d.Earr[0], Ez = d.Earr[nE - 1];
    unsigned int *flags = bar + 32, *flagsT = bar + 32 + 1024;
    unsigned long long *rows = reinterpret_cast<unsigned long long *>(d.partials);
    unsigned long long *Tpub = reinterpret_cast<unsigned long long *>(d.T_sv);
    const int NBP = (NB + 1) & ~1;
    unsigned long long *dbg = reinterpret_cast<unsigned long long *>(bar + 8);
#ifdef NK_STAMPS
    if (R > 0) nk_emit_segments<1, BOX>(d, L, step0, wg, G, false, 0ull, 0ull);
#else
    if (R > 0) nk_emit_segments<1, BOX>(d, L, step0, wg, G, false);
#endif
    for (int s = 0; s < nsteps; ++s) {
        const uint32_t step = step0 + (uint32_t)s;
        const int do_flux = (flux_every > 0 && ((step + 1u) % (uint32_t)flux_every) == 0u) ? 1 : 0;
        const bool mark = s == nsteps - 1 && tid == 0 && (wg == 0 || wg == G / 2);
        unsigned long long *mk = dbg + (wg == 0 ? 0 : 8);
        if (mark) mk[0] = __builtin_amdgcn_s_memrealtime();
#ifdef NK_STAMPS
        nk_sweep_body<1, false, false, PID, false, LREC, 0, BOX>(d, L, step, s == 0 ? relax0 : 1, do_flux, wg, G, 0ull);
#else
        nk_sweep_body<1, false, false, PID, false, LREC, 0, BOX>(d, L, step, s == 0 ? relax0 : 1, do_flux, wg, G);
#endif
        unsigned long long *rows_s = rows + (size_t)(s & 1) * G * NBP;
        __syncthreads();
        if (mark) mk[1] = __builtin_amdgcn_s_memrealtime();
        for (int b = tid; b < NB; b += NK_WG) {
            double v = 0.0;
            if (b < S) { for (int r = 0; r < NK_NREP; ++r) v += L.bins.E[r * S + b]; }
            else if (b < 2 * S) { unsigned int c = 0; for (int r = 0; r < NK_NREP; ++r) c += L.bins.N[r * S + (b - S)]; v = (double)c; }
            else if (b < 5 * S) { const int k = b - 2 * S; for (int r = 0; r < NK_NREP; ++r) v += L.bins.flux[r * 3 * S + k]; }
            else if (b < 5 * S + R) v = (double)L.bins.nleave[b - 5 * S];
            else if (b < 5 * S + 2 * R) v = L.bins.resb[4 * (b - 5 * S - R)];
            else if (b < 5 * S + 5 * R) { const int k = b - 5 * S - 2 * R; v = L.bins.resb[4 * (k / 3) + 1 + (k % 3)]; }
            else v = (double)L.bins.misc[0];
            __hip_atomic_store(rows_s + (size_t)wg * NBP + b, (unsigned long long)__double_as_longlong(v), __ATOMIC_RELAXED, __HIP_MEMORY_SCOPE_AGENT);
        }
        if (tid == 0 && NBP > NB) __hip_atomic_store(rows_s + (size_t)wg * NBP + NB, 0ull, __ATOMIC_RELAXED, __HIP_MEMORY_SCOPE_AGENT);
        asm volatile("s_waitcnt vmcnt(0) lgkmcnt(0)" ::: "memory");
        __builtin_amdgcn_fence(__ATOMIC_RELEASE, "workgroup");
        __syncthreads();
        if (tid == 0) __hip_atomic_store(flags + wg, (unsigned int)(s + 1), __ATOMIC_RELAXED, __HIP_MEMORY_SCOPE_AGENT);
        for (int i = tid; i < NK_NREP * S; i += NK_WG) { L.bins.E[i] = 0.0; L.bins.N[i] = 0u; }
        for (int i = tid; i < NK_NREP * 3 * S; i += NK_WG) L.bins.flux[i] = 0.0;
        for (int i = tid; i < 4 * R; i += NK_WG) L.bins.resb[i] = 0.0;
        for (int i = tid; i < R; i += NK_WG) L.bins.nleave[i] = 0u;
        if (tid == 0) L.bins.misc[0] = 0u;
        __syncthreads();
        if (mark && wg == 0) mk[2] = __builtin_amdgcn_s_memrealtime();
#ifdef NK_STAMPS
        if (R > 0 && s + 1 < nsteps) nk_emit_segments<1, BOX>(d, L, step + 1u, wg, G, true, 0ull, 0ull);
#else
        if (R > 0 && s + 1 < nsteps) nk_emit_segments<1, BOX>(d, L, step + 1u, wg, G, true);
#endif
        int ok = 1, hreq = 0;
        if (mark) mk[wg == 0 ? 3 : 2] = __builtin_amdgcn_s_memrealtime();
        double *hrowp = hist + (size_t)s * hrow;
        const int ntask = S + (NB - 2 * S);
        if (wg < ntask) {
            for (int g = tid; g < G; g += NK_WG) if (!nk_wait_word(flags + g, (unsigned int)(s + 1))) ok = 0;
            ok = __syncthreads_and(ok);
            if (!ok) {
                if (tid == 0) atomicOr(d.overflow, 256);
                return;
// ... 863 lines not shown
```

nanokappa_amd/engine.py:

```python
import ctypes as C
import os

import numpy as np

_HERE = os.path.dirname(os.path.abspath(__file__))
LIB_PATH = os.path.join(_HERE, os.environ.get('NK_LIBNAME', 'libnanokappa_hip.so'))

c_dp = C.POINTER(C.c_double)
c_ip = C.POINTER(C.c_int32)
c_bp = C.POINTER(C.c_int8)
c_up = C.POINTER(C.c_uint8)
c_u64p = C.POINTER(C.c_uint64)


class NkError(RuntimeError):
    pass


class nk_material(C.Structure):
    _fields_ = [('Q', C.c_int32), ('J', C.c_int32), ('NT', C.c_int32),
                ('omega', c_dp), ('group_vel', c_dp), ('T_grid', c_dp), ('lifetime', c_dp),
                ('nE', C.c_int32), ('T_fill_lo', C.c_double), ('T_fill_hi', C.c_double),
                ('T_array', c_dp), ('energy_array', c_dp),
                ('hbar', C.c_double), ('kb', C.c_double), ('QV', C.c_double), ('active_modes', C.c_int32)]


class nk_mesh(C.Structure):
    _fields_ = [('F', C.c_int32), ('normals', c_dp), ('k', c_dp), ('bounds_lo', c_dp), ('bounds_hi', c_dp),
                ('basis', c_dp), ('origins', c_dp), ('face_facet', c_ip), ('vertices', c_dp), ('face_area', c_dp),
                ('Fc', C.c_int32), ('facet_bc', c_bp), ('facet_partner', c_ip), ('facet_centroid', c_dp),
                ('facet_normal', c_dp), ('facet_face_off', c_ip), ('facet_face_idx', c_ip),
                ('tol', C.c_double), ('bbox', C.c_double * 6),
                ('nS', C.c_int32), ('simplex_pts', c_dp), ('simplex_vol', c_dp)]


class nk_subvols(C.Structure):
    _fields_ = [('S', C.c_int32), ('kind', C.c_int32), ('axis', C.c_int32), ('interp', C.c_int32),
                ('centers', c_dp), ('volumes', c_dp), ('rbf_inv', c_dp), ('rbf_shift', c_dp), ('rbf_scale', c_dp),
                ('rbf_used', C.c_int32 * 3)]


class nk_reservoirs(C.Structure):
    _fields_ = [('R', C.c_int32), ('facet', c_ip), ('T', c_dp), ('enter_prob', c_dp), ('counter', c_dp),
                ('gen', C.c_int32), ('n_leaving', C.POINTER(C.c_int64))]


class nk_rough(C.Structure):
    _fields_ = [('Fr', C.c_int32), ('facet', c_ip), ('specularity', c_dp), ('true_spec', c_up),
                ('spec_map', c_ip), ('roulette', c_dp), ('degen_j2', c_ip)]


class nk_params(C.Structure):
    _fields_ = [('dt', C.c_double), ('norm_fixed', C.c_int32), ('particle_density', C.c_double),
                ('T_ref_local', C.c_int32), ('T_ref', C.c_double), ('flux_every', C.c_int32),
                ('contains_every', C.c_int32), ('track_ids', C.c_int32)]


class nk_tally(C.Structure):
    _fields_ = [('T_sv', c_dp), ('E_sv', c_dp), ('E_raw', c_dp), ('N_sv', c_dp), ('flux_raw', c_dp),
                ('N_leaving', c_dp), ('res_energy', c_dp), ('res_flux', c_dp), ('N_emitted', c_dp)]


class nk_timing(C.Structure):
    _fields_ = [('step_kernel_ms', C.c_double), ('emit_kernel_ms', C.c_double), ('events_kernel_ms', C.c_double),
                ('total_ms', C.c_double),
                ('slots', C.c_int64), ('live', C.c_int64),
                ('regrows', C.c_int64), ('halts', C.c_int64), ('tau_rebuilds', C.c_int64), ('batches', C.c_int64),
                ('emit_fused', C.c_int64), ('place_tries', C.c_int64), ('place_gbps', C.c_double), ('place_worst_gbps', C.c_double),
                ('box_store', C.c_int64)]


class nk_comm_report(C.Structure):
    _fields_ = [('rank', C.c_int32), ('nranks', C.c_int32), ('comm_rank', C.c_int32), ('comm_nranks', C.c_int32),
                ('device', C.c_int32), ('selftest_ok', C.c_int32), ('selftest_sum', C.c_double), ('pci_bus_id', C.c_char * 32)]


EXPORTS = ['nk_device_count', 'nk_create', 'nk_destroy', 'nk_last_error', 'nk_set_material', 'nk_set_mesh', 'nk_set_subvolumes',
           'nk_set_reservoirs', 'nk_set_rough', 'nk_set_params', 'nk_reserve', 'nk_upload_particles',
           'nk_init_boundaries', 'nk_step', 'nk_download_particles', 'nk_get_subvol_temperature',
           'nk_set_subvol_temperature', 'nk_get_step', 'nk_get_timing', 'nk_comm_unique_id', 'nk_comm_init',
           'nk_find_boundary', 'nk_find_boundary_from', 'nk_tree_info', 'nk_classify', 'nk_box_hit', 'nk_eval', 'nk_mode_segments', 'nk_reflect', 'nk_uniform2', 'nk_calibrate_stream',
           'nk_specular_begin', 'nk_specular_pairs', 'nk_specular_end', 'nk_rough_begin', 'nk_rough_pairs', 'nk_rough_finish',
           'nk_rough_download', 'nk_build_enter_prob', 'nk_init_particles', 'nk_tally_state', 'nk_kspec_begin', 'nk_kspec_pairs',
           'nk_rough_finish_k', 'nk_mesh_crossings', 'nk_comm_info', 'nk_comm_allreduce', 'nk_set_bands', 'nk_get_band_rows',
           'nk_tally_bands_state', 'nk_set_field', 'nk_get_field', 'nk_tally_field_state', 'nk_field_info',
           'nk_set_field_groups', 'nk_get_field_groups', 'nk_tally_field_groups_state', 'nk_field_groups_info',
           'nk_set_modes', 'nk_get_modes', 'nk_tally_modes_state', 'nk_modes_info',
           'nk_group_create', 'nk_group_destroy', 'nk_group_step', 'nk_group_info', 'nk_group_last_error',
           'nk_cell_solid_volume', 'nk_solid_last_error', 'nk_free_paths', 'nk_free_paths_info', 'nk_free_paths_columns',
           'nk_free_paths_map', 'nk_free_paths_map_info', 'nk_kinetic_flights']

class nk_field(C.Structure):
    _fields_ = [('lo', C.c_double * 3), ('h', C.c_double * 3), ('n', C.c_int32 * 3), ('every', C.c_int32), ('flags', C.c_int32),
                ('capacity', C.c_int64)]


class nk_field_report(C.Structure):
    _fields_ = [('n', C.c_int32 * 3), ('every', C.c_int32), ('ncells', C.c_int64), ('k_E', C.c_int32), ('k_F', C.c_int32),
                ('B_E', C.c_double), ('B_F', C.c_double), ('capacity', C.c_int64), ('bytes', C.c_int64),
                ('lds_path', C.c_int32), ('on', C.c_int32)]


class nk_field_groups_report(C.Structure):
    _fields_ = [('G', C.c_int32), ('lds_path', C.c_int32), ('lines', C.c_int64), ('bytes', C.c_int64), ('k_E', C.c_int32),
                ('k_F', C.c_int32), ('permutes', C.c_int64), ('on', C.c_int32), ('pad_', C.c_int32)]


class nk_modes(C.Structure):
    _fields_ = [('every', C.c_int32), ('flags', C.c_int32), ('capacity', C.c_int64)]


class nk_modes_report(C.Structure):
    _fields_ = [('every', C.c_int32), ('k_E', C.c_int32), ('B_E', C.c_double), ('capacity', C.c_int64), ('bytes', C.c_int64),
                ('owner_path', C.c_int32), ('on', C.c_int32)]


class nk_tree_report(C.Structure):
    _fields_ = [('NG', C.c_int32), ('tree_top', C.c_int32), ('level_nodes', C.c_int32 * 8), ('tree_base', C.c_int32 * 8),
                ('top_family', C.c_int32), ('tree_leaves', C.c_int32), ('references', C.c_int32), ('pad_slots', C.c_int32),
                ('n_families', C.c_int32), ('pad_', C.c_int32), ('tree_bound', C.c_double)]


class nk_solid_report(C.Structure):
    _fields_ = [('ncells', C.c_int64), ('pairs', C.c_int64), ('k_A', C.c_int32), ('k_P', C.c_int32), ('seconds', C.c_double)]


class nk_free_path_args(C.Structure):
    _fields_ = [('n_modes', C.c_int32), ('modes', c_ip), ('n_samples', C.c_int32), ('max_segments', C.c_int32),
                ('w_min', C.c_double), ('tau', c_dp), ('x0', c_dp), ('seed', C.c_uint64)]


class nk_free_path_modes(C.Structure):
    _fields_ = [('D', c_dp), ('D2', c_dp), ('T', c_dp), ('hits', c_dp), ('p_res', c_dp), ('p_wall', c_dp), ('w_left', c_dp),
                ('p_int', c_dp)]


class nk_free_path_rays(C.Structure):
    _fields_ = [('D', c_dp), ('T', c_dp), ('segments', c_ip), ('end', c_ip), ('x0', c_dp)]


class nk_free_path_report(C.Structure):
    _fields_ = [('rays', C.c_int64), ('casts', C.c_int64), ('missed', C.c_int64), ('capped', C.c_int64),
                ('geometry_mode', C.c_int32), ('calls', C.c_int32), ('bytes', C.c_int64), ('seconds', C.c_double)]


FREE_PATH_MAX_COLUMNS = 32


class nk_free_path_columns_report(C.Structure):
    _fields_ = [('rays', C.c_int64), ('casts_shared', C.c_int64), ('casts', C.c_int64 * FREE_PATH_MAX_COLUMNS),
                ('missed', C.c_int64 * FREE_PATH_MAX_COLUMNS), ('capped', C.c_int64 * FREE_PATH_MAX_COLUMNS),
                ('n_columns', C.c_int32), ('tile', C.c_int32), ('launches', C.c_int32), ('geometry_mode', C.c_int32),
                ('calls', C.c_int32), ('pad_', C.c_int32), ('bytes', C.c_int64), ('seconds', C.c_double)]


FREE_MAP_LINE = 16


class nk_free_path_grid(C.Structure):
    _fields_ = [('n', C.c_int32 * 3), ('pad_', C.c_int32), ('lo', C.c_double * 3), ('h', C.c_double * 3), ('weight', c_dp),
                ('capacity', C.c_int64), ('weight_bound', C.c_double), ('ray_cell', c_ip), ('ray_w', c_dp)]


class nk_free_path_map_report(C.Structure):
    _fields_ = [('rays', C.c_int64), ('casts', C.c_int64), ('missed', C.c_int64), ('capped', C.c_int64), ('clamped', C.c_int64),
                ('overflow', C.c_int64), ('k_K', C.c_int32), ('k_P', C.c_int32), ('k_T', C.c_int32), ('geometry_mode', C.c_int32),
                ('calls', C.c_int32), ('pad_', C.c_int32), ('B_K', C.c_double), ('B_T', C.c_double), ('bytes', C.c_int64),
                ('seconds', C.c_double)]


KIN_MAX_SOURCES = 8
KIN_ROW_WORDS = 32


class nk_kinetic_args(C.Structure):
    _fields_ = [('n_samples', C.c_int32), ('max_events', C.c_int32), ('rays_per_wave', C.c_int32), ('no_bins', C.c_int32),
                ('tau', c_dp), ('cdf_scatter', c_dp), ('cdf_flux', c_dp), ('seed', C.c_uint64)]


class nk_kinetic_out(C.Structure):
    _fields_ = [('rows', C.POINTER(C.c_int64)), ('sub', C.POINTER(C.c_int64))]


class nk_kinetic_rays(C.Structure):
    _fields_ = [('x0', c_dp), ('mode', c_ip), ('end', c_ip), ('events', c_ip), ('casts', c_ip), ('D', c_dp), ('dwell', c_dp),
                ('hash', c_u64p)]


class nk_kinetic_report(C.Structure):
    _fields_ = [('rays', C.c_int64), ('events', C.c_int64), ('casts', C.c_int64), ('lost', C.c_int64), ('missed', C.c_int64),
                ('capped', C.c_int64), ('overflow', C.c_int64), ('n_sources', C.c_int32), ('n_subvolumes', C.c_int32),
                ('source_facet', C.c_int32 * KIN_MAX_SOURCES), ('k_D', C.c_int32), ('k_D2', C.c_int32), ('k_T', C.c_int32),
                ('k_t', C.c_int32), ('k_x', C.c_int32), ('geometry_mode', C.c_int32), ('lds_bins', C.c_int32), ('grid', C.c_int32),
                ('calls', C.c_int32), ('pad_', C.c_int32), ('B_t', C.c_double), ('B_x', C.c_double), ('bytes', C.c_int64),
                ('seconds', C.c_double)]


class nk_group_report(C.Structure):
    _fields_ = [('R', C.c_int32), ('halted', C.c_int32), ('finished_alone', C.c_int32), ('grid_sweep', C.c_int32),
                ('grid_tail', C.c_int32), ('pad_', C.c_int32), ('steps', C.c_int64), ('sweep_launches', C.c_int64),
                ('tail_launches', C.c_int64), ('member_launches', C.c_int64), ('sweep_kernel_ms', C.c_double),
                ('tail_kernel_ms', C.c_double), ('total_ms', C.c_double)]


ERR_ARG = -2
ERR_CAPACITY = -3
GROUP_MAX_MEMBERS = 32
MODES_GLOBAL = 1
MODES_TEST_SMALL_BOUND = 2
FIELD_GLOBAL = 1
FIELD_TEST_SMALL_BOUND = 2

_lib = None


def load_library():
    global _lib
    if _lib is not None:
        return _lib
    if not os.path.exists(LIB_PATH):
        raise NkError('%s not found: build it with `make -C %s` (needs hipcc); there is no CPU fallback'
                      % (LIB_PATH, os.path.join(_HERE, 'csrc')))
    L = C.CDLL(LIB_PATH)
    L.nk_last_error.restype = C.c_char_p
    L.nk_last_error.argtypes = [C.c_void_p]
    L.nk_create.argtypes = [C.POINTER(C.c_void_p), C.c_int, C.c_uint64]
    L.nk_destroy.argtypes = [C.c_void_p]
    L.nk_destroy.restype = None
    for name, st in (('nk_set_material', nk_material), ('nk_set_mesh', nk_mesh), ('nk_set_reservoirs', nk_reservoirs),
                     ('nk_set_rough', nk_rough), ('nk_set_params', nk_params)):
        getattr(L, name).argtypes = [C.c_void_p, C.POINTER(st)]
    L.nk_set_subvolumes.argtypes = [C.c_void_p, C.POINTER(nk_subvols), c_dp]
    L.nk_reserve.argtypes = [C.c_void_p, C.c_int64]
    L.nk_upload_particles.argtypes = [C.c_void_p, C.c_int64, c_dp, c_dp, c_dp, c_ip, c_dp, c_dp, c_ip, c_u64p, C.c_uint64]
    L.nk_init_boundaries.argtypes = [C.c_void_p]
    L.nk_init_particles.argtypes = [C.c_void_p, C.c_int64, C.c_int64, C.c_uint64, c_ip, C.c_int64, C.POINTER(C.c_int64)]
    L.nk_tally_state.argtypes = [C.c_void_p, c_dp, c_dp, c_dp]
    L.nk_mesh_crossings.argtypes = [C.c_int, C.c_int64, c_dp, c_dp, C.c_int64, c_dp, c_dp, c_dp, C.c_int, c_ip]
    L.nk_step.argtypes = [C.c_void_p, C.c_int32, C.POINTER(nk_tally)]
    L.nk_download_particles.argtypes = [C.c_void_p, C.c_int64, c_dp, c_dp, c_dp, c_ip, c_dp, c_dp, c_ip, c_u64p,
                                        C.POINTER(C.c_int64)]
    L.nk_get_subvol_temperature.argtypes = [C.c_void_p, c_dp]
    L.nk_set_subvol_temperature.argtypes = [C.c_void_p, c_dp]
    L.nk_get_step.argtypes = [C.c_void_p, C.POINTER(C.c_int64)]
    L.nk_get_timing.argtypes = [C.c_void_p, C.POINTER(nk_timing)]
    L.nk_comm_unique_id.argtypes = [C.c_void_p]
    L.nk_comm_init.argtypes = [C.c_void_p, C.c_void_p, C.c_int, C.c_int]
    L.nk_comm_info.argtypes = [C.c_void_p, C.POINTER(nk_comm_report)]
    L.nk_comm_allreduce.argtypes = [C.c_void_p, c_dp, C.c_int64]
    L.nk_find_boundary.argtypes = [C.c_void_p, C.c_int64, c_dp, c_dp, c_dp, c_dp, c_ip]
    L.nk_find_boundary_from.argtypes = [C.c_void_p, C.c_int64, c_dp, c_dp, c_ip, c_dp, c_dp, c_ip, c_ip]
    L.nk_tree_info.argtypes = [C.c_void_p, C.POINTER(nk_tree_report), C.POINTER(C.c_float), C.POINTER(C.c_float)]
    L.nk_classify.argtypes = [C.c_void_p, C.c_int64, c_dp, c_ip]
    L.nk_box_hit.argtypes = [C.c_void_p, C.c_int32, C.c_int64, c_dp, c_dp, c_dp, c_ip]
    L.nk_eval.argtypes = [C.c_void_p, C.c_int32, C.c_int64, c_dp, c_ip, c_dp]
    L.nk_mode_segments.argtypes = [C.c_void_p, c_ip, C.POINTER(C.c_int32)]
    L.nk_reflect.argtypes = [C.c_void_p, C.c_int64, c_ip, c_ip, c_dp, c_dp, c_dp, c_dp, c_dp, c_dp, c_ip, c_dp, c_dp]
    L.nk_uniform2.argtypes = [C.c_uint64, C.c_uint64, C.c_uint32, C.c_uint32, c_dp, c_dp]
    L.nk_calibrate_stream.argtypes = [C.c_void_p, C.c_int32, C.POINTER(C.c_int64), C.POINTER(C.c_int64)]
    L.nk_specular_begin.argtypes = [C.c_void_p, C.c_int64, c_dp, c_dp, c_dp]
    L.nk_specular_pairs.argtypes = [C.c_void_p, c_dp, C.c_double, C.c_int64, c_ip, c_ip, C.POINTER(C.c_int64)]
    L.nk_specular_end.argtypes = [C.c_void_p]
    L.nk_rough_begin.argtypes = [C.c_void_p, C.c_int32, c_ip, c_dp, c_dp, c_dp]
    L.nk_rough_pairs.argtypes = [C.c_void_p, C.c_int32, c_ip]
    L.nk_rough_finish.argtypes = [C.c_void_p]
    L.nk_rough_finish_k.argtypes = [C.c_void_p, C.c_int32, c_ip, c_ip]
    L.nk_kspec_begin.argtypes = [C.c_void_p, C.c_int64, c_dp, c_dp, c_dp, c_dp]
    L.nk_kspec_pairs.argtypes = [C.c_void_p, c_dp, C.c_int64, c_ip, c_ip, C.POINTER(C.c_int64)]
    L.nk_rough_download.argtypes = [C.c_void_p, c_dp, c_up, c_ip, c_dp]
    L.nk_build_enter_prob.argtypes = [C.c_void_p, C.c_int32, c_dp, c_dp, C.c_double, c_dp]
    L.nk_set_bands.argtypes = [C.c_void_p, C.c_int32, c_ip]
    L.nk_get_band_rows.argtypes = [C.c_void_p, c_dp, c_dp, C.POINTER(C.c_int64), C.c_int32, c_ip]
    L.nk_tally_bands_state.argtypes = [C.c_void_p, c_dp, c_dp]
    c_i64p = C.POINTER(C.c_int64)
    L.nk_set_field.argtypes = [C.c_void_p, C.POINTER(nk_field)]
    L.nk_get_field.argtypes = [C.c_void_p, c_dp, c_dp, c_dp, c_i64p, c_i64p, C.c_int32]
    L.nk_tally_field_state.argtypes = [C.c_void_p, c_i64p, c_i64p]
    L.nk_field_info.argtypes = [C.c_void_p, C.POINTER(nk_field_report)]
    L.nk_set_field_groups.argtypes = [C.c_void_p, C.c_int32, c_ip]
    L.nk_get_field_groups.argtypes = [C.c_void_p, c_dp, c_dp, c_dp, c_i64p, c_i64p, C.c_int32]
    L.nk_tally_field_groups_state.argtypes = [C.c_void_p, c_i64p, c_i64p, c_i64p]
    L.nk_field_groups_info.argtypes = [C.c_void_p, C.POINTER(nk_field_groups_report)]
    L.nk_set_modes.argtypes = [C.c_void_p, C.POINTER(nk_modes)]
    L.nk_get_modes.argtypes = [C.c_void_p, c_dp, c_dp, c_i64p, c_i64p, C.c_int32]
    L.nk_tally_modes_state.argtypes = [C.c_void_p, c_i64p, c_i64p]
    L.nk_modes_info.argtypes = [C.c_void_p, C.POINTER(nk_modes_report)]
    L.nk_group_create.argtypes = [C.POINTER(C.c_void_p), C.POINTER(C.c_void_p), C.c_int32]
    L.nk_group_destroy.argtypes = [C.c_void_p]
    L.nk_group_destroy.restype = None
    L.nk_group_step.argtypes = [C.c_void_p, C.c_int32, C.POINTER(nk_tally)]
    L.nk_group_info.argtypes = [C.c_void_p, C.POINTER(nk_group_report)]
    L.nk_group_last_error.restype = C.c_char_p
    L.nk_group_last_error.argtypes = [C.c_void_p]
    L.nk_cell_solid_volume.argtypes = [C.c_int, C.c_int64, c_dp, c_dp, c_dp, c_ip, c_dp, C.POINTER(nk_solid_report)]
    L.nk_solid_last_error.restype = C.c_char_p
    L.nk_solid_last_error.argtypes = []
    L.nk_free_paths.argtypes = [C.c_void_p, C.POINTER(nk_free_path_args), C.POINTER(nk_free_path_modes), C.POINTER(nk_free_path_rays),
                                C.POINTER(nk_free_path_report)]
    L.nk_free_paths_info.argtypes = [C.c_void_p, C.POINTER(nk_free_path_report)]
    L.nk_free_paths_map.argtypes = [C.c_void_p, C.POINTER(nk_free_path_args), C.POINTER(nk_free_path_grid), C.POINTER(C.c_int64),
                                    C.POINTER(nk_free_path_modes), C.POINTER(nk_free_path_rays), C.POINTER(nk_free_path_map_report)]
    L.nk_free_paths_map_info.argtypes = [C.c_void_p, C.POINTER(nk_free_path_map_report)]
    L.nk_free_paths_columns.argtypes = [C.c_void_p, C.POINTER(nk_free_path_args), C.c_int32, C.POINTER(nk_free_path_modes),
                                        C.POINTER(nk_free_path_rays), C.POINTER(nk_free_path_columns_report)]
    L.nk_kinetic_flights.argtypes = [C.c_void_p, C.POINTER(nk_kinetic_args), C.POINTER(nk_kinetic_out), C.POINTER(nk_kinetic_rays),
                                     C.POINTER(nk_kinetic_report)]
    _lib = L
    return L


def _d(a):
    return np.ascontiguousarray(a, dtype=np.float64)


def _i(a):
    return np.ascontiguousarray(a, dtype=np.int32)


def _p(a, t=c_dp):
    return None if a is None else a.ctypes.data_as(t)


def bc_codes(bound_cond):
    a = np.asarray(bound_cond)
    if a.dtype.kind in 'US':
        return np.array([ord(str(c)[0]) for c in a], dtype=np.int8)
    return np.ascontiguousarray(a, dtype=np.int8)

# ... 488 lines not shown

    def kinetic_flights(self, tau, c, n=65536, max_events=0, seed=0, rays=False, rays_per_wave=0, lds_bins=True):
        from . import kinetic as KN
        n = int(n)
        t, cc = _d(np.ravel(tau)), _d(np.ravel(c))
        if self.M > 0 and (t.shape[0] != self.M or cc.shape[0] != self.M):
            raise NkError('kinetic_flights: tau has %d and c %d entries, the material %d modes' % (t.shape[0], cc.shape[0], self.M))
        try:
            cs, cf = KN.tables(cc, t, self._vg)
        except ValueError as e:
            raise NkError('kinetic_flights: %s' % e)
        cs, cf = _d(cs), _d(cf)
        a = nk_kinetic_args()
        a.n_samples, a.max_events, a.rays_per_wave, a.no_bins = n, int(max_events), int(rays_per_wave), 0 if lds_bins else 1
        a.tau, a.cdf_scatter, a.cdf_flux, a.seed = _p(t), _p(cs), _p(cf), int(seed)
        F, S, nn = KIN_MAX_SOURCES, max(self.S, 1), max(n, 0)
        rows, sub = np.zeros((F, KIN_ROW_WORDS), dtype=np.int64), np.zeros(F * S * 4, dtype=np.int64)
        o = nk_kinetic_out()
        o.rows, o.sub = rows.ctypes.data_as(C.POINTER(C.c_int64)), sub.ctypes.data_as(C.POINTER(C.c_int64))
        pr, ro = None, {}
        if rays:
            ro = dict(ray_x0=np.zeros((F, nn, 3)), ray_mode=np.zeros((F, nn), dtype=np.int32), ray_end=np.zeros((F, nn), dtype=np.int32),
                      ray_events=np.zeros((F, nn), dtype=np.int32), ray_casts=np.zeros((F, nn), dtype=np.int32), ray_D=np.zeros((F, nn, 3)),
                      ray_dwell=np.zeros((F, nn)), ray_hash=np.zeros((F, nn), dtype=np.uint64))
            pr = nk_kinetic_rays()
            pr.x0, pr.D, pr.dwell = _p(ro['ray_x0']), _p(ro['ray_D']), _p(ro['ray_dwell'])
            pr.mode, pr.end, pr.events, pr.casts = (_p(ro[k], c_ip) for k in ('ray_mode', 'ray_end', 'ray_events', 'ray_casts'))
            pr.hash = _p(ro['ray_hash'], c_u64p)
        rep = nk_kinetic_report()
        rc = self.L.nk_kinetic_flights(self.h, C.byref(a), C.byref(o), C.byref(pr) if pr else None, C.byref(rep))
        r = {k: (list(getattr(rep, k)) if k == 'source_facet' else getattr(rep, k)) for k, _ in nk_kinetic_report._fields_ if k != 'pad_'}
        if rc != 0 and not (rc == ERR_CAPACITY and r['overflow'] > 0):
            self._ck(rc, 'nk_kinetic_flights')
        nf = int(rep.n_sources)
        r['source_facet'] = r['source_facet'][:nf]
        r['message'] = self.L.nk_last_error(self.h).decode() if rc != 0 else ''
        rows, sub = rows[:nf].copy(), sub[:nf * S * 4].reshape(nf, S, 4).copy()
        out = dict(n=n, source_facet=np.array(r['source_facet'], dtype=np.int32), ends=rows[:, :nf].copy(), lost=rows[:, 8].copy(),
                   missed=rows[:, 9].copy(), capped=rows[:, 10].copy(), events=rows[:, 11].copy(), casts=rows[:, 12].copy(),
                   D=rows[:, 13:16] * 2.0 ** -r['k_D'], D2=rows[:, 16:19] * 2.0 ** -r['k_D2'], dwell_total=rows[:, 19] * 2.0 ** -r['k_T'],
                   dwell=sub[:, :, 0] * 2.0 ** -r['k_t'], flux=sub[:, :, 1:4] * 2.0 ** -r['k_x'], rows=rows, sub=sub,
                   cdf_scatter=cs, cdf_flux=cf, report=r)
        for k, v in ro.items():
            out[k] = v[:nf].copy()
        return out

    def get_step(self):
        n = C.c_int64(0)
        self._ck(self.L.nk_get_step(self.h, C.byref(n)), 'nk_get_step')
        return int(n.value)

    def download(self):
        n = C.c_int64(0)
        self._ck(self.L.nk_download_particles(self.h, 0, None, None, None, None, None, None, None, None, C.byref(n)),
                 'nk_download_particles')
        N = int(n.value)
        x, y, z, occ, nts = (np.zeros(N) for _ in range(5))
        mode, facet = np.zeros(N, dtype=np.int32), np.zeros(N, dtype=np.int32)
        pid = np.zeros(N, dtype=np.uint64)
        if N:
            self._ck(self.L.nk_download_particles(self.h, N, _p(x), _p(y), _p(z), _p(mode, c_ip), _p(occ), _p(nts),
                                                  _p(facet, c_ip), _p(pid, c_u64p), C.byref(n)), 'nk_download_particles')
        return dict(positions=np.stack((x, y, z), axis=1), mode=mode, occupation=occ, n_timesteps=nts, facet=facet, pid=pid)

    def subvol_temperature(self):
        t = np.zeros(self.S)
        self._ck(self.L.nk_get_subvol_temperature(self.h, _p(t)), 'nk_get_subvol_temperature')
        return t

    def set_subvol_temperature(self, T):
        t = _d(T)
        self._ck(self.L.nk_set_subvol_temperature(self.h, _p(t)), 'nk_set_subvol_temperature')

    def timing(self):
        t = nk_timing()
        self._ck(self.L.nk_get_timing(self.h, C.byref(t)), 'nk_get_timing')
        return dict(step_kernel_ms=t.step_kernel_ms, emit_kernel_ms=t.emit_kernel_ms, events_kernel_ms=t.events_kernel_ms,
                    total_ms=t.total_ms,
                    slots=int(t.slots), live=int(t.live), regrows=int(t.regrows), halts=int(t.halts),
                    tau_rebuilds=int(t.tau_rebuilds), batches=int(t.batches), emit_fused=int(t.emit_fused),
                    place_tries=int(t.place_tries), place_gbps=t.place_gbps, place_worst_gbps=t.place_worst_gbps,
                    box_store=int(t.box_store))

    def specular_begin(self, group_vel, omega, delta_omega):
        v, om, dl = _d(np.asarray(group_vel).reshape(-1, 3)), _d(np.ravel(omega)), _d(np.ravel(delta_omega))
        self._ck(self.L.nk_specular_begin(self.h, om.shape[0], _p(v), _p(om), _p(dl)), 'nk_specular_begin')
        self._spec_M = om.shape[0]

    def specular_pairs(self, normal, crit=1e-3, download=True):
        nrm = _d(np.asarray(normal, dtype=float))
        cap = getattr(self, '_spec_cap', 4 * self._spec_M)
        while True:
            n = C.c_int64(0)
            if download:
                pi, po = np.empty(cap, dtype=np.int32), np.empty(cap, dtype=np.int32)
                self._ck(self.L.nk_specular_pairs(self.h, _p(nrm), float(crit), cap, _p(pi, c_ip), _p(po, c_ip), C.byref(n)),
                         'nk_specular_pairs')
            else:
                self._ck(self.L.nk_specular_pairs(self.h, _p(nrm), float(crit), cap, None, None, C.byref(n)), 'nk_specular_pairs')
            if n.value <= cap:
                return (pi[:n.value].astype(np.int64), po[:n.value].astype(np.int64)) if download else None
            cap = self._spec_cap = int(n.value)

    def specular_end(self):
        self._ck(self.L.nk_specular_end(self.h), 'nk_specular_end')

    def rough_begin(self, facets, normal_in, eta, k_norm):
        f, n, e, k = _i(facets), _d(normal_in), _d(eta), _d(k_norm)
        self._rough_Fr = f.shape[0]
        self._ck(self.L.nk_rough_begin(self.h, f.shape[0], _p(f, c_ip), _p(n), _p(e), _p(k)), 'nk_rough_begin')

    def rough_pairs(self, rough_facet_indices):
        f = _i(rough_facet_indices)
        self._ck(self.L.nk_rough_pairs(self.h, f.shape[0], _p(f, c_ip)), 'nk_rough_pairs')

    def rough_finish(self, degeneracies=None, degen_j2=None):
        if degeneracies is None:
            self._ck(self.L.nk_rough_finish(self.h), 'nk_rough_finish')
            return
        dg = _i(np.asarray(degeneracies, dtype=np.int32).reshape(-1, 3))
        dj = None if degen_j2 is None else _i(degen_j2)
        self._ck(self.L.nk_rough_finish_k(self.h, dg.shape[0], _p(dg, c_ip), _p(dj, c_ip)), 'nk_rough_finish_k')

    def kspec_begin(self, wavevectors, k_to_q, q_to_k, tol):
        kv, a, b, t = _d(wavevectors), _d(np.asarray(k_to_q, dtype=float).reshape(3, 3)), _d(np.asarray(q_to_k, dtype=float).reshape(3, 3)), _d(tol)
        self._ck(self.L.nk_kspec_begin(self.h, kv.shape[0], _p(kv), _p(a), _p(b), _p(t)), 'nk_kspec_begin')

    def kspec_pairs(self, normal, download=True):
        nrm = _d(np.asarray(normal, dtype=float))
        cap = self._spec_M
        n = C.c_int64(0)
        if download:
            pi, po = np.empty(cap, dtype=np.int32), np.empty(cap, dtype=np.int32)
            self._ck(self.L.nk_kspec_pairs(self.h, _p(nrm), cap, _p(pi, c_ip), _p(po, c_ip), C.byref(n)), 'nk_kspec_pairs')
            return pi[:n.value].astype(np.int64), po[:n.value].astype(np.int64)
        self._ck(self.L.nk_kspec_pairs(self.h, _p(nrm), cap, None, None, C.byref(n)), 'nk_kspec_pairs')
        return None

    def rough_download(self):
        Fr, M = self._rough_Fr, self.M
        sp, ts = np.zeros((Fr, M)), np.zeros((Fr, M), dtype=np.uint8)
        sm, ro = np.zeros((Fr, M), dtype=np.int32), np.zeros((Fr, M))
        self._ck(self.L.nk_rough_download(self.h, _p(sp), _p(ts, c_up), _p(sm, c_ip), _p(ro)), 'nk_rough_download')
        return sp, ts, sm, ro

    def build_enter_prob(self, normal_in, thickness, dt):
        n, t = _d(normal_in), _d(thickness)
        out = np.zeros((t.shape[0], self.M))
        self._ck(self.L.nk_build_enter_prob(self.h, t.shape[0], _p(n), _p(t), float(dt), _p(out)), 'nk_build_enter_prob')
        return out

    def calibrate_stream(self, launches=3):
        r, w = C.c_int64(0), C.c_int64(0)
        self._ck(self.L.nk_calibrate_stream(self.h, int(launches), C.byref(r), C.byref(w)), 'nk_calibrate_stream')
        return int(r.value), int(w.value)

    def comm_init(self, unique_id, rank, nranks):
        buf = C.create_string_buffer(bytes(unique_id), 128)
        self._ck(self.L.nk_comm_init(self.h, buf, int(rank), int(nranks)), 'nk_comm_init')

    def comm_allreduce(self, *arrays):
        flat = _d(np.concatenate([np.ravel(np.asarray(a, dtype=float)) for a in arrays]))
        self._ck(self.L.nk_comm_allreduce(self.h, _p(flat), flat.shape[0]), 'nk_comm_allreduce')
        out, off = [], 0
        for a in arrays:
            a = np.asarray(a)
# ... 132 lines not shown
```

Before: 53.13 billion.

## Precompute reservoir emissions for several future steps in a device ring buffer

Adds an emission ring. One build kernel generates reservoir newborn particles (positions, occupancy, ids, residual counters) for up to `depth` future steps in a single launch and stores them in a device buffer. Later steps then run only a cheap copy kernel that appends the prebuilt particles to the segment stores. This spreads the per-step emission work, including sampling and ray tracing, over a batch so it is paid less often. The cost is extra device memory, invalidation logic whenever the configuration changes, and wasted builds when a batch halts early. It only applies in single-rank, non-migration reservoir configurations.

```diff
diff --git a/include/nanokappa_hip.h b/include/nanokappa_hip.h
--- a/include/nanokappa_hip.h
+++ b/include/nanokappa_hip.h
@@ -160,6 +160,16 @@
 int nk_set_subvol_temperature(nk_ctx *ctx, const double *T_sv );
 int nk_get_step(nk_ctx *ctx, int64_t *step);
 int nk_get_timing(nk_ctx *ctx, nk_timing *t);
+typedef struct {
+    int64_t builds;
+    int64_t copies;
+    int64_t invalidations;
+    int64_t depth;
+    int64_t bytes;
+    int64_t first_step;
+    int64_t last_step;
+} nk_emit_ring_report;
+int nk_emit_ring_info(nk_ctx *ctx, nk_emit_ring_report *out);
 
 int nk_comm_unique_id(void *id128 );
 int nk_comm_init(nk_ctx *ctx, const void *id128, int rank, int nranks);
diff --git a/nanokappa_amd/csrc/nk_engine.hip b/nanokappa_amd/csrc/nk_engine.hip
--- a/nanokappa_amd/csrc/nk_engine.hip
+++ b/nanokappa_amd/csrc/nk_engine.hip
@@ -22,6 +22,7 @@
 #include "nk_field.h"
 #include "nk_modes.h"
 #include "nk_group.h"
+#include "nk_ring.h"
 #include "nk_freepath.h"
 #include "nk_freecols.h"
 #include "nk_kinetic.h"
@@ -49,6 +50,17 @@
 
 static thread_local std::string g_create_error;
 
+struct NkRingHost {
+    NkRing g = {};
+    void *buf = nullptr;
+    size_t bytes = 0;
+    int depth = 0;
+    bool ok = false;
+    int64_t base = 0, last = -1;
+    bool carved = false;
+    int nseg = 0, nlmax = 0;
+    int64_t builds = 0, copies = 0, invalidations = 0;
+};
 struct nk_ctx {
     int device = 0;
     hipStream_t stream = nullptr;
@@ -103,6 +115,7 @@
     void *inbox = nullptr, *inbox_n = nullptr;
     void *mig_buf = nullptr, *mig_n = nullptr;
     double *ep_p = nullptr, *rc_p = nullptr;
+    NkRingHost ring;
     int rm_nseg = 0, rm_nlmax = 0;
     int32_t halt_words[4] = {0, 0, 0, 0};
     double *acc = nullptr;
@@ -396,6 +409,7 @@
     if (ctx->mig_n) hipFree(ctx->mig_n);
     if (ctx->ep_p) hipFree(ctx->ep_p);
     if (ctx->rc_p) hipFree(ctx->rc_p);
+    if (ctx->ring.buf) hipFree(ctx->ring.buf);
     if (ctx->band_map) hipFree(ctx->band_map);
     if (ctx->band_slabs) hipFree(ctx->band_slabs);
     if (ctx->band_rows_d) hipFree(ctx->band_rows_d);
@@ -406,8 +420,16 @@
     delete ctx;
 }
 
+static void nk_ring_invalidate(nk_ctx *ctx) {
+    if (!ctx) return;
+    if (ctx->ring.ok) ctx->ring.invalidations += 1;
+    ctx->ring.ok = false;
+    ctx->ring.carved = false;
+}
+
 int nk_set_material(nk_ctx *ctx, const nk_material *m) {
     if (ctx) ctx->emitted_for = -1;
+    nk_ring_invalidate(ctx);
     NK_ARG(ctx && m, "nk_set_material: NULL argument");
     NK_ARG(m->Q > 0 && m->J > 0 && m->NT >= 2 && m->nE >= 2, "nk_set_material: bad sizes");
     NK_HIP(hipSetDevice(ctx->device));
@@ -483,6 +505,7 @@
 
 int nk_set_mesh(nk_ctx *ctx, const nk_mesh *m) {
     if (ctx) ctx->emitted_for = -1;
+    nk_ring_invalidate(ctx);
     NK_ARG(ctx && m, "nk_set_mesh: NULL argument");
     NK_ARG(m->F > 0 && m->Fc > 0, "nk_set_mesh: empty mesh");
     NK_HIP(hipSetDevice(ctx->device));
@@ -826,6 +849,7 @@
 
 static int nk_entry_tables_drop(nk_ctx *ctx, bool keep_counters) {
     NkDev &d = ctx->d;
+    nk_ring_invalidate(ctx);
     if (ctx->rm_nseg > 0 && keep_counters && d.R > 0 && d.res_counter) {
         const int64_t n = (int64_t)d.R * d.M;
         k_perm_rm<<<(int)((n + 255) / 256), 256, 0, ctx->stream>>>(0, d.R, d.M, ctx->rm_nseg, ctx->rm_nlmax,
@@ -930,6 +954,7 @@
 
 int nk_set_reservoirs(nk_ctx *ctx, const nk_reservoirs *r) {
     if (ctx) ctx->emitted_for = -1;
+    nk_ring_invalidate(ctx);
     NK_ARG(ctx && r, "nk_set_reservoirs: NULL argument");
     NK_ARG(ctx->have_material && ctx->have_mesh && ctx->have_sv, "nk_set_reservoirs: set material, mesh, subvolumes first");
     NK_ARG(r->R >= 0 && r->R <= 64, "nk_set_reservoirs: R must be in [0, 64]");
@@ -1045,6 +1070,7 @@
 
 int nk_set_params(nk_ctx *ctx, const nk_params *p) {
     if (ctx) ctx->emitted_for = -1;
+    nk_ring_invalidate(ctx);
     NK_ARG(ctx && p, "nk_set_params: NULL argument");
     NK_ARG(p->dt > 0, "nk_set_params: dt must be positive");
     ctx->params = *p;
@@ -1257,6 +1283,7 @@
     d.m2s = nullptr; d.s2m = nullptr; d.seg_nl = nullptr;
     ctx->h_m2s.clear(); ctx->h_s2m.clear(); ctx->map_nseg = 0;
     ctx->map_gen += 1;
+    nk_ring_invalidate(ctx);
     if (d.M <= 0 || d.nseg <= 0) return NK_OK;
     const int M = d.M, nseg = d.nseg, nlmax = d.nlmax;
     const bool plain = !d.part;
@@ -2070,11 +2097,64 @@
     return NK_OK;
 }
 
+#define NK_RING_MAX_DEPTH 32
+#define NK_RING_MAX_BYTES ((size_t)1 << 30)
+static inline int nk_ring_depth() {
+    const char *e = getenv("NK_EMIT_RING");
+    const int v = e ? atoi(e) : 8;
+    return v < 2 ? 0 : (v > NK_RING_MAX_DEPTH ? NK_RING_MAX_DEPTH : v);
+}
+static inline bool nk_ring_wanted(const nk_ctx *ctx, const NkBatch &b) {
+    const NkDev &d = ctx->d;
+    return b.tail_emit && !ctx->comm && (d.res_gen == 0 || d.res_gen == 1) && nk_geom_mode(ctx) == 1 && !d.qx && !d.mig_buf && d.Fr == 0 &&
+           d.ep_p && d.nseg > 0 && !ctx->h_enter_prob.empty() && nk_ring_depth() >= 2;
+}
+static bool nk_ring_carve(nk_ctx *ctx) {
+    NkDev &d = ctx->d;
+    NkRingHost &rg = ctx->ring;
+    const int depth = nk_ring_depth();
+    if (rg.carved && rg.depth == depth && rg.nseg == d.nseg && rg.nlmax == d.nlmax && (rg.g.pid != nullptr) == (bool)d.pid &&
+        (rg.g.nts != nullptr) == (bool)d.nts) return true;
+    if (rg.ok) rg.invalidations += 1;
+    rg.ok = false; rg.carved = false;
+    std::vector<int64_t> per((size_t)d.nseg, 0);
+    for (int r = 0; r < d.R; ++r)
+        for (int m = 0; m < d.M; ++m)
+            per[(size_t)nk_mode_seg(ctx, m, d.nseg)] += ((int64_t)floor(ctx->h_enter_prob[(size_t)r * d.M + m]) + 1 + d.nranks - 1) / d.nranks;
+    int64_t mx = 1;
+    for (int64_t v : per) mx = std::max(mx, v);
+    const size_t rcap = (size_t)((mx + NK_TILE - 1) / NK_TILE) * NK_TILE, slots = (size_t)(depth - 1) * d.nseg * rcap;
+    const size_t nd = 4 + (d.nts ? 1 : 0) + (d.pid ? 1 : 0);
+    const size_t bytes = slots * (nd * 8 + 4) + (size_t)(depth - 1) * d.nseg * 8 + (d.res_gen == 0 ? (size_t)(depth - 1) * d.rc_len * 8 : 0) + 64;
+    if (bytes > NK_RING_MAX_BYTES || rcap >= ((size_t)1 << 24)) return false;
+    if (bytes > rg.bytes) {
+        if (rg.buf) hipFree(rg.buf);
+        rg.buf = nullptr; rg.bytes = 0;
+        if (hipMalloc(&rg.buf, bytes) != hipSuccess) { (void)hipGetLastError(); rg.buf = nullptr; return false; }
+        rg.bytes = bytes;
+    }
+    double *p = (double *)rg.buf;
+    rg.g.x = p; p += slots; rg.g.y = p; p += slots; rg.g.z = p; p += slots; rg.g.occ = p; p += slots;
+    rg.g.nts = nullptr; rg.g.pid = nullptr; rg.g.rc = nullptr;
+    if (d.nts) { rg.g.nts = p; p += slots; }
+    if (d.pid) { rg.g.pid = (uint64_t *)p; p += slots; }
+    if (d.res_gen == 0) { rg.g.rc = p; p += (size_t)(depth - 1) * d.rc_len; }
+    rg.g.hdr = (int32_t *)p; p += (size_t)(depth - 1) * d.nseg;
+    rg.g.w0 = (uint32_t *)p;
+    rg.g.rcap = (int32_t)rcap;
+    rg.depth = depth; rg.nseg = d.nseg; rg.nlmax = d.nlmax;
+    rg.carved = true;
+    return true;
+}
+
 static int nk_step_batch(nk_ctx *ctx, int32_t nsteps, std::vector<double> &h, int32_t *done) {
     NkDev &d = ctx->d;
     const int R = d.R, NB = d.NB;
     NkBatch b;
     NK_TRY(nk_batch_enter(ctx, nsteps, b));
+    NkRingHost &rg = ctx->ring;
+    const bool ring = nk_ring_wanted(ctx, b) && nk_ring_carve(ctx);
+    int ring_built = -1;
     const size_t lds_g = nk_lds(ctx, true), lds_w = nk_lds(ctx, true, d.pid ? 3 : 2), lds_e = nk_lds(ctx, true, 1), lds_t = nk_tail_lds(ctx);
     const size_t lds_ev = nk_events_lds(ctx, lds_g);
     const NkSweepKind kind = nk_sweep_kind(ctx, true);
@@ -2123,6 +2203,17 @@
             ncclResult_t nrc = ctx->rccl.AllReduce(ctx->acc, ctx->acc, (size_t)NB + 2, ncclDouble, ncclSum, ctx->comm, ctx->stream);
             if (nrc != ncclSuccess) { ctx->err = "ncclAllReduce failed"; return NK_ERR_COMM; }
             k_update<<<1, NK_WG, 0, ctx->stream>>>(d, ctx->acc, hrow, do_flux);
+        } else if (ahead && ring) {
+            const int64_t n = ctx->step + s + 1;
+            if (rg.ok && n > rg.base && n <= rg.last) {
+                NK_HIP(nk_ring_launch_copy(NB + g_emit, ctx->stream, d, rg.g, step + 1u, (int)(n - rg.base - 1), rows, ctx->acc, hrow, do_flux, NB));
+                rg.copies += 1;
+            } else {
+                NK_HIP(nk_ring_launch_build(d.box != 0, NB + g_emit, lds_t, ctx->stream, d, rg.g, step + 1u, rg.depth, rows, ctx->acc, hrow, do_flux, NB));
+                rg.ok = true; rg.base = n; rg.last = n + rg.depth - 1;
+                rg.builds += 1;
+                ring_built = s;
+            }
         } else if (ahead) {
             NK_EMIT_LAUNCH(k_tail, NB + g_emit, lds_t, d, step + 1u, rows, ctx->acc, hrow, do_flux, 1, NB);
         } else {
@@ -2141,6 +2232,11 @@
 #endif
     NK_TRY(nk_band_collect(ctx, band_s, *done));
     nk_batch_leave(ctx, b, nsteps, *done);
+    if (ring_built >= 0) {
+        const int32_t *hw_ = ctx->halt_words;
+        const bool halted = *done < nsteps || hw_[0] || hw_[2] || hw_[3];
+        if (ring_built >= *done || (ring_built == *done - 1 && halted)) { rg.ok = false; rg.builds -= 1; }
+    }
     return nk_batch_timing(ctx, nev, nsteps, *done);
 }
 
@@ -2707,6 +2803,16 @@
     t->box_store = (ctx->d.cap > 0 && ctx->d.box) ? 1 : 0;
     return NK_OK;
 }
+int nk_emit_ring_info(nk_ctx *ctx, nk_emit_ring_report *out) {
+    NK_ARG(ctx && out, "nk_emit_ring_info: NULL argument");
+    const NkRingHost &rg = ctx->ring;
+    out->builds = rg.builds; out->copies = rg.copies; out->invalidations = rg.invalidations;
+    out->depth = nk_ring_depth();
+    out->bytes = (int64_t)rg.bytes;
+    out->first_step = rg.ok ? rg.base + 1 : 0;
+    out->last_step = rg.ok ? rg.last : -1;
+    return NK_OK;
+}
 
 static int nk_load_rccl(NkRccl &r, std::string &err) {
     if (r.lib) return NK_OK;
@@ -2736,6 +2842,7 @@
 }
 int nk_comm_init(nk_ctx *ctx, const void *id128, int rank, int nranks) {
     if (ctx) ctx->emitted_for = -1;
+    nk_ring_invalidate(ctx);
     NK_ARG(ctx && id128 && nranks >= 1 && rank >= 0 && rank < nranks, "nk_comm_init: bad arguments");
     NK_ARG(!ctx->stepped, "nk_comm_init: must be called before the first nk_step (emission ownership is per rank)");
     NK_HIP(hipSetDevice(ctx->device));
diff --git a/nanokappa_amd/csrc/nk_kernels.h b/nanokappa_amd/csrc/nk_kernels.h
--- a/nanokappa_amd/csrc/nk_kernels.h
+++ b/nanokappa_amd/csrc/nk_kernels.h
@@ -1404,6 +1404,196 @@
     }
 }
 
+struct NkRing {
+    double *x, *y, *z, *occ, *nts;
+    uint64_t *pid;
+    uint32_t *w0;
+    int32_t *hdr;
+    double *rc;
+    int32_t rcap;
+};
+
+template <bool BOX>
+__device__ __forceinline__ void nk_ring_build_one(const NkDev &d, const NkLds &L, const NkRing &g, uint32_t step, int nb, int seg, int lane,
+                                                  unsigned int *sp_pref, unsigned int *sp_cnt, unsigned int *sp_rm, double *sp_cv, double *sp_pr) {
+    const int plo = d.seg_lo ? d.seg_lo[seg] : 0;
+    const int64_t base = (int64_t)seg * d.segcap;
+    const int count = d.seg_count[seg];
+    const NkSegModes sm = nk_seg_modes(d, seg);
+    const int nent = d.R * sm.nl;
+    int made_v = 0;
+    int sp_bound = 0;
+    for (int e0 = 0; e0 < nent; e0 += NK_EMIT_CHUNK) {
+        double e_prob[2], e_cnt[2];
+        int64_t e_at[2];
+        unsigned int e_rm[2], e_rl[2];
+#pragma unroll
+        for (int k = 0; k < 2; ++k) {
+            const int e = e0 + k * 64 + lane;
+            e_prob[k] = 0.0; e_cnt[k] = 0.0; e_at[k] = -1; e_rm[k] = 0u; e_rl[k] = 0u;
+            if (e < nent) {
+                const int r = e / sm.nl, l = e - r * sm.nl;
+                e_rl[k] = ((unsigned int)r << 12) | ((unsigned int)l << 18);
+                e_rm[k] = (unsigned int)((int64_t)r * d.M + sm.entry_mode(l));
+                e_at[k] = ((int64_t)seg * d.R + r) * d.nlmax + l;
+                e_prob[k] = d.ep_p[e_at[k]];
+                if (d.res_gen == 0) e_cnt[k] = d.rc_p[(int64_t)(step & 1u) * d.rc_len + e_at[k]];
+                sp_bound += ((int)floor(e_prob[k]) + 1 + d.nranks - 1) / d.nranks;
+            }
+        }
+        for (int s = 0; s < nb; ++s) {
+            const uint32_t st = step + (uint32_t)s;
+            unsigned int run = 0;
+#pragma unroll
+            for (int k = 0; k < 2; ++k) {
+                int c = 0, cmine = 0;
+                double cv = 0.0;
+                if (e_at[k] >= 0) {
+                    const double prob = e_prob[k], fixed = floor(prob);
+                    int mask;
+                    if (d.res_gen == 0) {
+                        cv = e_cnt[k] + (prob - fixed);
+                        mask = cv >= 1.0;
+                        cv -= (double)mask;
+                        e_cnt[k] = cv;
+                        if (s == 0) d.rc_p[(int64_t)((st + 1u) & 1u) * d.rc_len + e_at[k]] = cv;
+                        else g.rc[(int64_t)(s - 1) * d.rc_len + e_at[k]] = cv;
+                    } else {
+                        double d1;
+                        nk_uniform2_dev(d.seed, (uint64_t)e_rm[k] | 0xFFFFFFFF00000000ull, st, NK_TAG_DICE, cv, d1);
+                        mask = cv <= (prob - fixed);
+                    }
+                    c = (int)fixed + mask;
+                    cmine = c;
+                    if (d.nranks > 1) {
+                        cmine = 0;
+                        for (int level = c; level >= 1; --level)
+                            cmine += ((e_rm[k] + (uint32_t)level + st) % (uint32_t)d.nranks) == (uint32_t)d.rank;
+                    }
+                }
+                unsigned int v = (unsigned int)cmine;
+#pragma unroll
+                for (int o = 1; o < 64; o <<= 1) { const unsigned int u = __shfl_up(v, o, 64); if (lane >= o) v += u; }
+                sp_cnt[k * 64 + lane] = (unsigned int)c | e_rl[k];
+                sp_rm[k * 64 + lane] = e_rm[k];
+                sp_cv[k * 64 + lane] = cv;
+                sp_pr[k * 64 + lane] = e_prob[k];
+                sp_pref[k * 64 + lane] = v + run - (unsigned int)cmine;
+                run += __shfl(v, 63, 64);
+            }
+            __builtin_amdgcn_fence(__ATOMIC_SEQ_CST, "wavefront");
+            const int spn = (int)run;
+            const int made = __shfl(made_v, s, 64);
+            const int64_t ring0 = s > 0 ? ((int64_t)(s - 1) * d.nseg + seg) * g.rcap : 0;
+            for (int spj = 0; spj < spn; spj += NK_TILE) {
+                const int j = spj + lane;
+                if (j >= spn) continue;
+                int lo = 0, hi = NK_EMIT_CHUNK;
+                while (hi - lo > 1) { const int mid = (lo + hi) >> 1; if ((int)sp_pref[mid] <= j) lo = mid; else hi = mid; }
+                const unsigned int cw = sp_cnt[lo];
+                const int q = j - (int)sp_pref[lo], c = (int)(cw & 0xFFFu);
+                const int r = (int)((cw >> 12) & 0x3Fu);
+                const int64_t rm = (int64_t)sp_rm[lo];
+                const int idx = d.part ? (int)(cw >> 18) : (int)((uint32_t)rm - (uint32_t)r * (uint32_t)d.M);
+                const double cval = sp_cv[lo], prob = sp_pr[lo];
+                int level;
+                if (d.nranks == 1) level = c - q;
+                else {
+                    const uint32_t n = (uint32_t)d.nranks;
+                    const uint32_t tq = ((uint32_t)d.rank + n - (((uint32_t)rm + st) % n)) % n;
+                    const uint32_t top = (uint32_t)c - (((uint32_t)c + n - tq) % n);
+                    level = (int)(top - (uint32_t)q * n);
+                }
+                const NkMode *rec = sm.rec + idx;
+                const double4 ra = *reinterpret_cast<const double4 *>(rec);
+                const double E0 = rec->E0;
+                const uint64_t pid = level > 0 ? ((uint64_t)((st + 1u) & 0xFFFFFFu) << 40) | ((uint64_t)rm << 12) | (uint64_t)level
+                                               : ((uint64_t)((st + 1u) & 0xFFFFFFu) << 40) | ((uint64_t)r << 32);
+                double uf, us, ur, ut;
+                nk_uniform2_dev(d.seed, pid, st, NK_TAG_EMIT, uf, us);
+                nk_uniform2_dev(d.seed, pid, st, NK_TAG_EMIT + 1, ur, ut);
+                const double iprob = level > 0 ? nk_rcp(prob) : 0.0;
+                const double dt_in = (level == 0) ? d.dt * ut
+                                   : (level == 1) ? d.dt * (1.0 - cval * iprob)
+                                                  : d.dt * (1.0 - ((double)(level - 1) + ut) * iprob);
+                double x0, y0, z0;
+                if (d.res_lds) nk_sample_res_face(L.rf_off, L.rf_cdf, L.rf_verts, r, uf, us, ur, x0, y0, z0);
+                else nk_sample_res_face(d.res_face_off, d.res_face_cdf, d.res_face_verts, r, uf, us, ur, x0, y0, z0);
+                const double omega = ra.x, vx = ra.y, vy = ra.z, vz = ra.w;
+                const double occ = nk_be(omega * d.c_hk, E0, L.resT[2 * r + 1], d.invT0);
+                double tc = 0.0;
+                int facet = -1;
+                if (!BOX) NK_RAY(1, d, L, NK_TREE_NO_SKIP, x0, y0, z0, vx, vy, vz, tc, facet);
+                double xa, ya, za, na;
+                nk_newborn_place(d, x0, y0, z0, vx, vy, vz, dt_in, tc, xa, ya, za, na);
+                const uint32_t w = BOX ? (NK_NEWBORN | (uint32_t)idx) : (NK_NEWBORN | ((uint32_t)(facet + 1) << d.lb) | (uint32_t)idx);
+                if (s == 0) {
+                    const int o = count + made + j;
+                    if (plo + o < d.segcap) {
+                        const NkSlot p = nk_slot(d, base + plo + o);
+                        d.x.p[p.od] = xa; d.y.p[p.od] = ya; d.z.p[p.od] = za;
+                        d.occ.p[p.od] = occ;
+                        if (!BOX) d.nts.p[p.od] = na;
+                        d.w0.p[p.ow] = w;
+                        if (d.pid) d.pid.p[p.od] = pid;
+                    } else if (!d.halt[1]) atomicOr(d.overflow, 1);
+                } else if (made + j < g.rcap) {
+                    const int64_t i = ring0 + made + j;
+                    g.x[i] = xa; g.y[i] = ya; g.z[i] = za;
+                    g.occ[i] = occ;
+                    if (!BOX) g.nts[i] = na;
+                    g.w0[i] = w;
+                    if (g.pid) g.pid[i] = pid;
+                }
+            }
+            if (lane == s) made_v += spn;
+            __builtin_amdgcn_fence(__ATOMIC_SEQ_CST, "wavefront");
+        }
+    }
+#pragma unroll
+    for (int o = 32; o > 0; o >>= 1) sp_bound += __shfl_xor(sp_bound, o, 64);
+    const int room = d.segcap - plo - count;
+    if (lane == 0) {
+        d.seg_new[seg] = made_v < room ? made_v : (room > 0 ? room : 0);
+        d.seg_bound[seg] = sp_bound;
+    } else if (lane < nb) {
+        int32_t *h = g.hdr + ((int64_t)(lane - 1) * d.nseg + seg) * 2;
+        h[0] = made_v < g.rcap ? made_v : g.rcap;
+        h[1] = sp_bound;
+    }
+}
+
+__device__ __forceinline__ void nk_ring_copy_one(const NkDev &d, const NkRing &g, uint32_t step, int k, int seg, int lane) {
+    const int plo = d.seg_lo ? d.seg_lo[seg] : 0;
+    const int64_t base = (int64_t)seg * d.segcap;
+    const int count = d.seg_count[seg];
+    const int nent = d.res_gen == 0 ? d.R * d.seg_nl[seg] : 0, nl = d.seg_nl[seg];
+    const int32_t *h = g.hdr + ((int64_t)k * d.nseg + seg) * 2;
+    const int made = h[0] < 0 ? 0 : (h[0] < g.rcap ? h[0] : g.rcap), bound = h[1];
+    const int64_t ring0 = ((int64_t)k * d.nseg + seg) * g.rcap;
+    const int room = d.segcap - plo - count;
+    const int put = made < room ? made : (room > 0 ? room : 0);
+    for (int j = lane; j < put; j += 64) {
+        const NkSlot p = nk_slot(d, base + plo + count + j);
+        const int64_t i = ring0 + j;
+        d.x.p[p.od] = g.x[i]; d.y.p[p.od] = g.y[i]; d.z.p[p.od] = g.z[i];
+        d.occ.p[p.od] = g.occ[i];
+        if (g.nts) d.nts.p[p.od] = g.nts[i];
+        d.w0.p[p.ow] = g.w0[i];
+        if (g.pid) d.pid.p[p.od] = g.pid[i];
+    }
+    for (int e = lane; e < nent; e += 64) {
+        const int r = e / nl, l = e - r * nl;
+        const int64_t at = ((int64_t)seg * d.R + r) * d.nlmax + l;
+        d.rc_p[(int64_t)((step + 1u) & 1u) * d.rc_len + at] = g.rc[(int64_t)k * d.rc_len + at];
+    }
+    if (lane == 0) {
+        if (put < made && !d.halt[1]) atomicOr(d.overflow, 1);
+        d.seg_new[seg] = put;
+        d.seg_bound[seg] = bound;
+    }
+}
+
 __device__ __forceinline__ bool nk_wait_word(const unsigned int *w, unsigned int atleast) {
     int spins = 0;
     while (__hip_atomic_load(w, __ATOMIC_RELAXED, __HIP_MEMORY_SCOPE_AGENT) < atleast) {
diff --git a/nanokappa_amd/csrc/nk_ring.h b/nanokappa_amd/csrc/nk_ring.h
--- /dev/null
+++ b/nanokappa_amd/csrc/nk_ring.h
@@ -0,0 +1,11 @@
+#pragma once
+#include <hip/hip_runtime.h>
+#include <stdint.h>
+
+struct NkDev;
+struct NkRing;
+
+hipError_t nk_ring_launch_build(bool box, int grid, size_t lds, hipStream_t stream, const NkDev &d, const NkRing &g, uint32_t step_next, int nb,
+                                int rows, double *acc, double *hist_row, int do_flux, int n_reduce);
+hipError_t nk_ring_launch_copy(int grid, hipStream_t stream, const NkDev &d, const NkRing &g, uint32_t step_next, int k, int rows, double *acc,
+                               double *hist_row, int do_flux, int n_reduce);
diff --git a/nanokappa_amd/csrc/nk_ring.hip b/nanokappa_amd/csrc/nk_ring.hip
--- /dev/null
+++ b/nanokappa_amd/csrc/nk_ring.hip
@@ -0,0 +1,52 @@
+#include <hip/hip_runtime.h>
+#include <stdint.h>
+#include "../../include/nanokappa_hip.h"
+#define NK_KERNEL_LINKAGE template <int NK_NOT_IN_THIS_TU = 0>
+#include "nk_kernels.h"
+#include "nk_ring.h"
+
+template <bool BOX>
+__global__ __launch_bounds__(NK_WG) void k_tail_ring(NkDev d, NkRing g, uint32_t step_next, int nb, int rows, double *acc, double *hist_row,
+                                                     int do_flux, int fuse, int n_reduce) {
+    extern __shared__ __align__(16) unsigned char smem[];
+    if ((int)blockIdx.x < n_reduce) {
+        double *sh = reinterpret_cast<double *>(smem);
+        int &last = *reinterpret_cast<int *>(smem + NK_WG * sizeof(double));
+        nk_reduce_body(d, rows, acc, hist_row, do_flux, fuse, (int)blockIdx.x, n_reduce, sh, last);
+        return;
+    }
+    if (d.halt[0]) return;
+    NkLds L;
+    nk_lds_setup<1, 1>(d, smem, L);
+    const int lane = threadIdx.x & 63, wave = __builtin_amdgcn_readfirstlane(threadIdx.x >> 6);
+    const int nwaves = ((int)gridDim.x - n_reduce) * (NK_WG / 64);
+    for (int seg = ((int)blockIdx.x - n_reduce) * (NK_WG / 64) + wave; seg < d.nseg; seg += nwaves)
+        nk_ring_build_one<BOX>(d, L, g, step_next, nb, seg, lane, L.sp_pref + wave * NK_EMIT_CHUNK, L.sp_cnt + wave * NK_EMIT_CHUNK,
+                               L.sp_rm + wave * NK_EMIT_CHUNK, L.sp_cv + wave * NK_EMIT_CHUNK, L.sp_pr + wave * NK_EMIT_CHUNK);
+}
+__global__ __launch_bounds__(NK_WG) void k_tail_copy(NkDev d, NkRing g, uint32_t step_next, int k, int rows, double *acc, double *hist_row,
+                                                     int do_flux, int fuse, int n_reduce) {
+    extern __shared__ __align__(16) unsigned char smem[];
+    if ((int)blockIdx.x < n_reduce) {
+        double *sh = reinterpret_cast<double *>(smem);
+        int &last = *reinterpret_cast<int *>(smem + NK_WG * sizeof(double));
+        nk_reduce_body(d, rows, acc, hist_row, do_flux, fuse, (int)blockIdx.x, n_reduce, sh, last);
+        return;
+    }
+    if (d.halt[0]) return;
+    const int lane = threadIdx.x & 63, wave = __builtin_amdgcn_readfirstlane(threadIdx.x >> 6);
+    const int nwaves = ((int)gridDim.x - n_reduce) * (NK_WG / 64);
+    for (int seg = ((int)blockIdx.x - n_reduce) * (NK_WG / 64) + wave; seg < d.nseg; seg += nwaves) nk_ring_copy_one(d, g, step_next, k, seg, lane);
+}
+
+hipError_t nk_ring_launch_build(bool box, int grid, size_t lds, hipStream_t stream, const NkDev &d, const NkRing &g, uint32_t step_next, int nb,
+                                int rows, double *acc, double *hist_row, int do_flux, int n_reduce) {
+    if (box) k_tail_ring<true><<<grid, NK_WG, lds, stream>>>(d, g, step_next, nb, rows, acc, hist_row, do_flux, 1, n_reduce);
+    else k_tail_ring<false><<<grid, NK_WG, lds, stream>>>(d, g, step_next, nb, rows, acc, hist_row, do_flux, 1, n_reduce);
+    return hipSuccess;
+}
+hipError_t nk_ring_launch_copy(int grid, hipStream_t stream, const NkDev &d, const NkRing &g, uint32_t step_next, int k, int rows, double *acc,
+                               double *hist_row, int do_flux, int n_reduce) {
+    k_tail_copy<<<grid, NK_WG, NK_WG * 8 + 16, stream>>>(d, g, step_next, k, rows, acc, hist_row, do_flux, 1, n_reduce);
+    return hipSuccess;
+}
diff --git a/nanokappa_amd/engine.py b/nanokappa_amd/engine.py
--- a/nanokappa_amd/engine.py
+++ b/nanokappa_amd/engine.py
@@ -68,6 +68,11 @@
                 ('regrows', C.c_int64), ('halts', C.c_int64), ('tau_rebuilds', C.c_int64), ('batches', C.c_int64),
                 ('emit_fused', C.c_int64), ('place_tries', C.c_int64), ('place_gbps', C.c_double), ('place_worst_gbps', C.c_double),
                 ('box_store', C.c_int64)]
+
+
+class nk_emit_ring_report(C.Structure):
+    _fields_ = [('builds', C.c_int64), ('copies', C.c_int64), ('invalidations', C.c_int64), ('depth', C.c_int64),
+                ('bytes', C.c_int64), ('first_step', C.c_int64), ('last_step', C.c_int64)]
 
 
 class nk_comm_report(C.Structure):
@@ -88,7 +93,7 @@
            'nk_set_modes', 'nk_get_modes', 'nk_tally_modes_state', 'nk_modes_info',
            'nk_group_create', 'nk_group_destroy', 'nk_group_step', 'nk_group_info', 'nk_group_last_error',
            'nk_cell_solid_volume', 'nk_solid_last_error', 'nk_free_paths', 'nk_free_paths_info', 'nk_free_paths_columns',
-           'nk_free_paths_map', 'nk_free_paths_map_info', 'nk_kinetic_flights']
+           'nk_free_paths_map', 'nk_free_paths_map_info', 'nk_kinetic_flights', 'nk_emit_ring_info']
 
 class nk_field(C.Structure):
     _fields_ = [('lo', C.c_double * 3), ('h', C.c_double * 3), ('n', C.c_int32 * 3), ('every', C.c_int32), ('flags', C.c_int32),
@@ -244,6 +249,7 @@
     L.nk_set_subvol_temperature.argtypes = [C.c_void_p, c_dp]
     L.nk_get_step.argtypes = [C.c_void_p, C.POINTER(C.c_int64)]
     L.nk_get_timing.argtypes = [C.c_void_p, C.POINTER(nk_timing)]
+    L.nk_emit_ring_info.argtypes = [C.c_void_p, C.POINTER(nk_emit_ring_report)]
     L.nk_comm_unique_id.argtypes = [C.c_void_p]
     L.nk_comm_init.argtypes = [C.c_void_p, C.c_void_p, C.c_int, C.c_int]
     L.nk_comm_info.argtypes = [C.c_void_p, C.POINTER(nk_comm_report)]
@@ -898,6 +904,11 @@
                     place_tries=int(t.place_tries), place_gbps=t.place_gbps, place_worst_gbps=t.place_worst_gbps,
                     box_store=int(t.box_store))
 
+    def emit_ring_info(self):
+        r = nk_emit_ring_report()
+        self._ck(self.L.nk_emit_ring_info(self.h, C.byref(r)), 'nk_emit_ring_info')
+        return {k: int(getattr(r, k)) for k, _ in nk_emit_ring_report._fields_}
+
     def specular_begin(self, group_vel, omega, delta_omega):
         v, om, dl = _d(np.asarray(group_vel).reshape(-1, 3)), _d(np.ravel(omega)), _d(np.ravel(delta_omega))
         self._ck(self.L.nk_specular_begin(self.h, om.shape[0], _p(v), _p(om), _p(dl)), 'nk_specular_begin')
```

Result: slower. 49.27 billion (-7.3%).
